# edouardoyallon/acco

Hardware: NVIDIA H100
Metric: tokens/sec (device-timed, max over ranks) Llama ACCO bf16 sharded-Adam, 8x1024 tokens per GPU per micro-batch (higher is better)
Workload: dtype bf16

## Files before the change

### acco_b200/csrc/bindings.cpp

```cpp
#include <torch/extension.h>
#include <ATen/cuda/CUDAContext.h>
#include <c10/cuda/CUDAGuard.h>
#include <cuda_runtime.h>

#include <cmath>
#include <cstdlib>
#include <vector>

extern "C" {
int acco_norm_grid(int T, int H, int sms, int backward);
int acco_norm_fwd(const void* a, const void* r, const void* w, const void* b, void* y, void* h, float* mean, float* rstd, int T, int H,
                  float eps, int grid, cudaStream_t st);
int acco_norm_bwd(const void* dy, const void* dh_extra, const void* h, const void* w, const float* mean, const float* rstd, void* dh,
                  float* partial, float* dwdb_out, void* dw_accum, void* db_accum, int T, int H, int grid, cudaStream_t st);
int acco_rope_pack_bwd(const void* dq, const void* dk, const void* dv, const long long* strides, void* dqkv, const float* cos_t,
                       const float* sin_t, int B, int S, int Hq, int Hk, int D, int sms, cudaStream_t st);
int acco_rope_qkv(void* qkv, const float* cos_t, const float* sin_t, int T, int S, int n_rot, int n_total, int D, int inverse,
                  int sms, cudaStream_t st);
int acco_swiglu_fwd(const void* gu, void* out, long long T, int I, int sms, cudaStream_t st);
int acco_swiglu_bwd(const void* dout, const void* gu, void* dgu, long long T, int I, int sms, cudaStream_t st);
int acco_ce_fwd(const void* logits, const long long* labels, float* lse, float* row_loss, float* loss, float* inv_n, long long T,
                int V, int Vp, long long ignore_index, cudaStream_t st);
int acco_ce_bwd(void* logits, const long long* labels, const float* lse, const float* scale, long long T, int V, int Vp,
                long long ignore_index, cudaStream_t st);
int acco_gelu_fwd(const void* x, void* y, long long n, int sms, cudaStream_t st);
int acco_gelu_bwd(const void* dy, const void* x, void* dx, long long n, int sms, cudaStream_t st);
int acco_debug_occupy(unsigned long long ns, int ctas, float* sink, cudaStream_t st);
int acco_round_params_size();
int acco_gemm_run(const void* a, long long lda, int a_mn, const void* b, long long ldb, int b_mn, void* d, long long ldd, const void* bias,
                  int M, int N, int K, int accumulate, int bn_req, int splits_req, int pm_req, int pn_req, int msub_req, int sms, cudaStream_t st);
int acco_gemm_tn_gather(const void* x, const void* w_local, void* y, int M, int N, int K, const void* const* peers, int n_peers,
                        const int* tile_owner, uint32_t* flags, uint32_t* epoch, uint32_t* done, int sms, cudaStream_t st);
long long acco_gemm_map_encodes();
int acco_gemm_max_clusters(int cl, int sms);
void acco_gemm_set_debug(unsigned long long* buf);
void acco_gemm_choose(int M, int N, int K, int a_mn, int b_mn, int accumulate, int sms, int* out5);
int acco_gemm_fp8_run(const void* a, long long lda, const void* b, long long ldb, void* d, long long ldd, const void* bias, int M, int N, int K,
                      int accumulate, int a_e5m2, const float* inv_a, const float* inv_b, int bn_req, int splits_req, int sms, cudaStream_t st);
int acco_fp8_amax_ctas(long long n, int sms);
int acco_fp8_quantize(const void* t, int R, int C, int e5m2, void* q, void* qT, float* scale_out, int ctas, cudaStream_t st);
int acco_gemm_tile_n();
int acco_gemm_tile_k();
int acco_attn_supported(int B, int S, int Hq, int Hk, int D, float scale);
int acco_attn_fwd(const void* q, const void* k, const void* v, long long ld, void* o, long long ld_o, float* lse, int B, int S, int Hq, int Hk,
                  int D, float scale, int window, const int* seg, cudaStream_t st);
int acco_attn_bwd(const void* q, const void* k, const void* v, long long ld, const void* o, long long ld_o, const void* d_o, long long ld_do,
                  const float* lse, float* delta, float* dq_acc, void* dk, void* dv, int B, int S, int Hq, int Hk, int D, float scale, int window,
                  const int* seg, cudaStream_t st);
}

namespace {

constexpr int kMaxWorld = 16;
struct RoundParams {
    const void* acc_peer[kMaxWorld];
    void* theta_peer[kMaxWorld];
    uint32_t* pad_peer[kMaxWorld];
    const void* acc_mc;
    void* theta_mc;
    float* master;
    float* exp_avg;
    float* exp_avg_sq;
    float* stash;
    int* stash_count;
    int* total_out;
    uint32_t* epoch;
    uint32_t* done_ctas;
    const float* inv_count_in;
    const long long* skip;
    int n_skip;
    int watchdog_s;
    int gated;
    long long slice;
    int rank, world, local_count;
    float lr, beta1, beta2, eps, weight_decay, bc1, bc2_rsqrt;
    int commit, add_stash, write_stash;
};
extern "C" int acco_rs_adam_ag(const RoundParams* P, int grad_bf16, int out_bf16, int mode, int grid, cudaStream_t st);
extern "C" int acco_round_norm(const RoundParams* P, int grad_bf16, int mode, int grid, float max_norm, float* out, cudaStream_t st);

int sm_count() {
    static int n = 0;
    if (!n) n = at::cuda::getCurrentDeviceProperties()->multiProcessorCount;
    return n;
}
cudaStream_t stream() { return at::cuda::getCurrentCUDAStream().stream(); }

void check_bf16(const torch::Tensor& t, const char* name) {
    TORCH_CHECK(t.is_cuda() && t.scalar_type() == torch::kBFloat16 && t.is_contiguous(), name, " must be a contiguous CUDA bf16 tensor");
}
void check_f32(const torch::Tensor& t, const char* name) {
    TORCH_CHECK(t.is_cuda() && t.scalar_type() == torch::kFloat32 && t.is_contiguous(), name, " must be a contiguous CUDA fp32 tensor");
}

std::vector<torch::Tensor> norm_fwd(torch::Tensor a, c10::optional<torch::Tensor> r, torch::Tensor w, c10::optional<torch::Tensor> b,
                                    double eps) {
    check_bf16(a, "a"); check_bf16(w, "weight");
    const bool has_r = r.has_value() && r->defined(), layer = b.has_value() && b->defined();
    if (has_r) check_bf16(*r, "r");
    if (layer) check_bf16(*b, "bias");
    const c10::cuda::CUDAGuard guard(a.device());
    const int T = a.size(0), H = a.size(1);
    TORCH_CHECK(w.numel() == H && (!layer || b->numel() == H), "norm: weight/bias size");
    auto y = torch::empty_like(a);
    auto f32 = a.options().dtype(torch::kFloat32);
    auto rstd = torch::empty({T}, f32);
    torch::Tensor mean = layer ? torch::empty({T}, f32) : torch::Tensor();
    torch::Tensor h = has_r ? torch::empty_like(a) : torch::Tensor();
    const int grid = acco_norm_grid(T, H, sm_count(), 0);
    TORCH_CHECK(acco_norm_fwd(a.data_ptr(), has_r ? r->data_ptr() : nullptr, w.data_ptr(), layer ? b->data_ptr() : nullptr, y.data_ptr(),
                              has_r ? h.data_ptr() : nullptr, layer ? mean.data_ptr<float>() : nullptr, rstd.data_ptr<float>(), T, H,
                              (float)eps, grid, stream()) == 0,
                "norm_fwd: unsupported hidden size ", H);
    return {y, h, mean, rstd};
}

std::vector<torch::Tensor> norm_bwd(torch::Tensor dy, c10::optional<torch::Tensor> dh_extra, torch::Tensor h, torch::Tensor w,
                                    c10::optional<torch::Tensor> mean, torch::Tensor rstd, c10::optional<torch::Tensor> wgrad,
                                    c10::optional<torch::Tensor> bgrad) {
    check_bf16(dy, "dy"); check_bf16(h, "h"); check_bf16(w, "weight"); check_f32(rstd, "rstd");
    const bool has_e = dh_extra.has_value() && dh_extra->defined(), layer = mean.has_value() && mean->defined();
    if (has_e) check_bf16(*dh_extra, "dh_extra");
    if (layer) check_f32(*mean, "mean");
    const c10::cuda::CUDAGuard guard(dy.device());
    const int T = dy.size(0), H = dy.size(1), np = layer ? 2 : 1;
    auto dh = torch::empty_like(dy);
    const int grid = acco_norm_grid(T, H, sm_count(), 1);
    auto f32 = dy.options().dtype(torch::kFloat32);
    auto partial = torch::empty({grid, np * H}, f32);
    const bool accum = wgrad.has_value() && wgrad->defined() && (!layer || (bgrad.has_value() && bgrad->defined()));
    torch::Tensor dwdb;
    if (accum) {
        check_bf16(*wgrad, "weight.grad");
        TORCH_CHECK(wgrad->numel() == H, "weight.grad has the wrong size");
        if (layer) {
            check_bf16(*bgrad, "bias.grad");
            TORCH_CHECK(bgrad->numel() == H, "bias.grad has the wrong size");
        }
        dwdb = torch::empty({0}, f32);
    } else {
        dwdb = torch::empty({np * H}, f32);
    }
    TORCH_CHECK(acco_norm_bwd(dy.data_ptr(), has_e ? dh_extra->data_ptr() : nullptr, h.data_ptr(), w.data_ptr(),
                              layer ? mean->data_ptr<float>() : nullptr, rstd.data_ptr<float>(), dh.data_ptr(), partial.data_ptr<float>(),
                              accum ? nullptr : dwdb.data_ptr<float>(), accum ? wgrad->data_ptr() : nullptr,
                              accum && layer ? bgrad->data_ptr() : nullptr, T, H, grid, stream()) == 0,
                "norm_bwd: unsupported hidden size ", H);
    return {dh, dwdb};
}

torch::Tensor gelu_fwd(torch::Tensor x) {
    check_bf16(x, "x");
    const c10::cuda::CUDAGuard guard(x.device());
    auto y = torch::empty_like(x);
    TORCH_CHECK(acco_gelu_fwd(x.data_ptr(), y.data_ptr(), x.numel(), sm_count(), stream()) == 0, "gelu: numel must be a multiple of 8");
    return y;
}
torch::Tensor gelu_bwd(torch::Tensor dy, torch::Tensor x) {
    check_bf16(x, "x"); check_bf16(dy, "dy");
    const c10::cuda::CUDAGuard guard(x.device());
    auto dx = torch::empty_like(x);
    TORCH_CHECK(acco_gelu_bwd(dy.data_ptr(), x.data_ptr(), dx.data_ptr(), x.numel(), sm_count(), stream()) == 0, "gelu: numel must be a multiple of 8");
    return dx;
}

void rope_qkv_inplace(torch::Tensor qkv, torch::Tensor cos_t, torch::Tensor sin_t, int64_t B, int64_t S, int64_t n_rot,
                      int64_t n_total, int64_t D, bool inverse) {
    check_bf16(qkv, "qkv"); check_f32(cos_t, "cos"); check_f32(sin_t, "sin");
    const c10::cuda::CUDAGuard guard(qkv.device());
    TORCH_CHECK(qkv.numel() == B * S * n_total * D, "qkv has the wrong number of elements");
    TORCH_CHECK(cos_t.size(0) >= S && cos_t.size(1) == D / 2, "cos/sin tables must be [>=S, D/2]");
    TORCH_CHECK(acco_rope_qkv(qkv.data_ptr(), cos_t.data_ptr<float>(), sin_t.data_ptr<float>(), (int)(B * S), (int)S, (int)n_rot,
                              (int)n_total, (int)D, inverse ? 1 : 0, sm_count(), stream()) == 0,
                "rope: head_dim must be a multiple of 16");
}

torch::Tensor rope_pack_bwd(torch::Tensor dq, torch::Tensor dk, torch::Tensor dv, torch::Tensor cos_t, torch::Tensor sin_t) {
    TORCH_CHECK(dq.is_cuda() && dq.scalar_type() == torch::kBFloat16 && dk.scalar_type() == torch::kBFloat16 && dv.scalar_type() == torch::kBFloat16, "bf16 CUDA grads expected");
    TORCH_CHECK(dq.stride(3) == 1 && dk.stride(3) == 1 && dv.stride(3) == 1, "head dim must be contiguous");
    check_f32(cos_t, "cos"); check_f32(sin_t, "sin");
    const c10::cuda::CUDAGuard guard(dq.device());
    const int64_t B = dq.size(0), S = dq.size(1), Hq = dq.size(2), D = dq.size(3), Hk = dk.size(2);
    for (auto* t : {&dq, &dk, &dv}) TORCH_CHECK((t->stride(0) % 8 == 0) && (t->stride(1) % 8 == 0) && (t->stride(2) % 8 == 0) && ((uintptr_t)t->data_ptr() % 16 == 0), "16-byte aligned strides required");
    auto out = torch::empty({B * S, (Hq + 2 * Hk) * D}, dq.options());
    long long st[9] = {dq.stride(0), dq.stride(1), dq.stride(2), dk.stride(0), dk.stride(1), dk.stride(2), dv.stride(0), dv.stride(1), dv.stride(2)};
    TORCH_CHECK(acco_rope_pack_bwd(dq.data_ptr(), dk.data_ptr(), dv.data_ptr(), st, out.data_ptr(), cos_t.data_ptr<float>(), sin_t.data_ptr<float>(),
                                   (int)B, (int)S, (int)Hq, (int)Hk, (int)D, sm_count(), stream()) == 0, "rope_pack_bwd: head_dim must be a multiple of 16");
    return out;
}

torch::Tensor swiglu_fwd(torch::Tensor gu) {
    check_bf16(gu, "gate_up");
    const c10::cuda::CUDAGuard guard(gu.device());
    const int64_t T = gu.size(0), I = gu.size(1) / 2;
    auto out = torch::empty({T, I}, gu.options());
    TORCH_CHECK(acco_swiglu_fwd(gu.data_ptr(), out.data_ptr(), T, (int)I, sm_count(), stream()) == 0, "swiglu: I must be a multiple of 8");
    return out;
}

torch::Tensor swiglu_bwd(torch::Tensor dout, torch::Tensor gu) {
    check_bf16(dout, "dout"); check_bf16(gu, "gate_up");
    const c10::cuda::CUDAGuard guard(gu.device());
    const int64_t T = gu.size(0), I = gu.size(1) / 2;
    auto dgu = torch::empty_like(gu);
    TORCH_CHECK(acco_swiglu_bwd(dout.data_ptr(), gu.data_ptr(), dgu.data_ptr(), T, (int)I, sm_count(), stream()) == 0, "swiglu: I must be a multiple of 8");
    return dgu;
}

std::vector<torch::Tensor> ce_fwd(torch::Tensor logits, torch::Tensor labels, int64_t V, int64_t ignore_index) {
    check_bf16(logits, "logits");
    TORCH_CHECK(labels.is_cuda() && labels.scalar_type() == torch::kInt64 && labels.is_contiguous(), "labels must be contiguous CUDA int64");
    const c10::cuda::CUDAGuard guard(logits.device());
    const int64_t T = logits.size(0), Vp = logits.size(1);
    TORCH_CHECK(labels.numel() == T, "labels/logits row mismatch");
    auto f32 = logits.options().dtype(torch::kFloat32);
    auto lse = torch::empty({T}, f32);
    auto row_loss = torch::empty({T}, f32);
    auto loss = torch::empty({}, f32);
    auto inv_n = torch::empty({1}, f32);
    TORCH_CHECK(acco_ce_fwd(logits.data_ptr(), (const long long*)labels.data_ptr<int64_t>(), lse.data_ptr<float>(), row_loss.data_ptr<float>(),
                            loss.data_ptr<float>(), inv_n.data_ptr<float>(), T, (int)V, (int)Vp, ignore_index, stream()) == 0,
                "ce_fwd: padded vocab must be a multiple of 8 and >= V");
    return {loss, inv_n, lse};
}

void ce_bwd_inplace(torch::Tensor logits, torch::Tensor labels, torch::Tensor lse, torch::Tensor scale, int64_t V, int64_t ignore_index) {
    check_bf16(logits, "logits"); check_f32(lse, "lse"); check_f32(scale, "scale");
    const c10::cuda::CUDAGuard guard(logits.device());
    const int64_t T = logits.size(0), Vp = logits.size(1);
    TORCH_CHECK(acco_ce_bwd(logits.data_ptr(), (const long long*)labels.data_ptr<int64_t>(), lse.data_ptr<float>(), scale.data_ptr<float>(), T,
                            (int)V, (int)Vp, ignore_index, stream()) == 0, "ce_bwd: bad shapes");
}

int default_grid(int mode, long long slice) {
    const long long vec = slice / 8;
    long long want = (vec + 255) / 256;
    long long cap = mode == 0 ? (long long)sm_count() * 4 : (long long)sm_count();
    if (want < 1) want = 1;
    return (int)std::min(want, cap);
}

void fill_hyper(RoundParams& P, double lr, double b1, double b2, double eps, double wd, int64_t step, int64_t commit, bool add_stash, bool write_stash) {
    P.lr = (float)lr; P.beta1 = (float)b1; P.beta2 = (float)b2; P.eps = (float)eps; P.weight_decay = (float)wd;
    P.bc1 = (float)(1.0 - std::pow(b1, (double)step));
    P.bc2_rsqrt = (float)(1.0 / std::sqrt(1.0 - std::pow(b2, (double)step)));
    P.commit = (int)commit; P.add_stash = add_stash ? 1 : 0; P.write_stash = write_stash ? 1 : 0;
}

void adamw_shard(torch::Tensor grad_sum, torch::Tensor master, torch::Tensor exp_avg, torch::Tensor exp_avg_sq, torch::Tensor stash,
                 torch::Tensor out, torch::Tensor inv_count, torch::Tensor scratch ,
                 double lr, double b1, double b2, double eps, double wd, int64_t step, int64_t commit, bool add_stash, bool write_stash) {
    check_f32(master, "master"); check_f32(exp_avg, "exp_avg"); check_f32(exp_avg_sq, "exp_avg_sq"); check_f32(stash, "stash"); check_f32(inv_count, "inv_count");
    const c10::cuda::CUDAGuard guard(master.device());
    const int64_t S = master.numel();
    TORCH_CHECK(S % 8 == 0, "shard size must be a multiple of 8 (use slice alignment >= 8)");
    TORCH_CHECK(grad_sum.numel() >= S && out.numel() >= S && grad_sum.is_contiguous() && out.is_contiguous(), "bad grad/out");
    TORCH_CHECK(scratch.scalar_type() == torch::kInt32 && scratch.numel() >= 4, "scratch must be int32[4]");
    const bool gb = grad_sum.scalar_type() == torch::kBFloat16, ob = out.scalar_type() == torch::kBFloat16;
    TORCH_CHECK(gb || grad_sum.scalar_type() == torch::kFloat32, "grad dtype");
    TORCH_CHECK(ob || out.scalar_type() == torch::kFloat32, "out dtype");
    RoundParams P{};
    P.acc_peer[0] = grad_sum.data_ptr();
    P.theta_peer[0] = out.data_ptr();
    P.master = master.data_ptr<float>(); P.exp_avg = exp_avg.data_ptr<float>(); P.exp_avg_sq = exp_avg_sq.data_ptr<float>(); P.stash = stash.data_ptr<float>();
    int* sc = scratch.data_ptr<int>();
    P.stash_count = sc; P.total_out = sc + 1; P.epoch = (uint32_t*)(sc + 2); P.done_ctas = (uint32_t*)(sc + 3);
    P.inv_count_in = inv_count.data_ptr<float>();
    P.slice = S; P.rank = 0; P.world = 1; P.local_count = 0;
    fill_hyper(P, lr, b1, b2, eps, wd, step, commit, add_stash, write_stash);
    TORCH_CHECK(acco_rs_adam_ag(&P, gb, ob, 0, default_grid(0, S), stream()) == 0, "adamw_shard launch failed");
}

RoundParams round_params(const std::vector<int64_t>& acc_ptrs, const std::vector<int64_t>& theta_ptrs, const std::vector<int64_t>& pad_ptrs,
                         int64_t acc_mc, int64_t theta_mc, const torch::Tensor& stash, const torch::Tensor& scratch, int64_t slice, int64_t rank,
                         int64_t world, int64_t local_count, int64_t mode) {
    check_f32(stash, "stash");
    TORCH_CHECK(world >= 1 && world <= kMaxWorld, "world size out of range");
    TORCH_CHECK(mode >= 0 && mode <= 2, "mode must be 0 (local), 1 (p2p) or 2 (multimem)");
    TORCH_CHECK((int64_t)acc_ptrs.size() >= (mode == 0 ? 1 : world), "peer pointer table too short");
    TORCH_CHECK(mode == 0 || (int64_t)pad_ptrs.size() >= world, "signal pad table too short");
    TORCH_CHECK(slice % 8 == 0 && stash.numel() == slice, "slice must be a multiple of 8 and match the shard state");
    TORCH_CHECK(mode != 2 || acc_mc != 0, "multicast mode needs multicast pointers");
    TORCH_CHECK(scratch.scalar_type() == torch::kInt32 && scratch.numel() >= 4, "scratch must be int32[4]");
    RoundParams P{};
    for (size_t i = 0; i < acc_ptrs.size() && i < (size_t)kMaxWorld; ++i) P.acc_peer[i] = (const void*)acc_ptrs[i];
    for (size_t i = 0; i < theta_ptrs.size() && i < (size_t)kMaxWorld; ++i) P.theta_peer[i] = (void*)theta_ptrs[i];
    for (size_t i = 0; i < pad_ptrs.size() && i < (size_t)kMaxWorld; ++i) P.pad_peer[i] = (uint32_t*)pad_ptrs[i];
    P.acc_mc = (const void*)acc_mc; P.theta_mc = (void*)theta_mc;
    P.stash = stash.data_ptr<float>();
    int* sc = scratch.data_ptr<int>();
    P.stash_count = sc; P.total_out = sc + 1; P.epoch = (uint32_t*)(sc + 2); P.done_ctas = (uint32_t*)(sc + 3);
    P.inv_count_in = nullptr;
    P.slice = slice; P.rank = (int)rank; P.world = (int)world; P.local_count = (int)local_count;
    static int watchdog = -1;
    if (watchdog < 0) { const char* e = std::getenv("ACCO_ROUND_WATCHDOG_S"); watchdog = e ? std::atoi(e) : 1800; }
    P.watchdog_s = watchdog;
    static int gated = -1;
    if (gated < 0) { const char* e = std::getenv("ACCO_ROUND_GATE"); gated = (e && e[0] == '0') ? 0 : 1; }
    P.gated = mode != 0 ? gated : 0;
    return P;
}

void rs_adam_ag(std::vector<int64_t> acc_ptrs, std::vector<int64_t> theta_ptrs, std::vector<int64_t> pad_ptrs, int64_t acc_mc, int64_t theta_mc,
                torch::Tensor master, torch::Tensor exp_avg, torch::Tensor exp_avg_sq, torch::Tensor stash,
                torch::Tensor scratch , int64_t slice, int64_t rank, int64_t world, int64_t local_count,
                double lr, double b1, double b2, double eps, double wd, int64_t step, int64_t commit, bool add_stash, bool write_stash,
                bool grad_bf16, bool out_bf16, int64_t mode, int64_t grid, c10::optional<torch::Tensor> skip_ranges,
                c10::optional<torch::Tensor> inv_count) {
    check_f32(master, "master"); check_f32(exp_avg, "exp_avg"); check_f32(exp_avg_sq, "exp_avg_sq");
    const c10::cuda::CUDAGuard guard(master.device());
    TORCH_CHECK(master.numel() == slice, "slice must match the shard state");
    TORCH_CHECK((int64_t)theta_ptrs.size() >= (mode == 0 ? 1 : world), "peer pointer tables too short");
    TORCH_CHECK(mode != 2 || theta_mc != 0, "multicast mode needs multicast pointers");
    RoundParams P = round_params(acc_ptrs, theta_ptrs, pad_ptrs, acc_mc, theta_mc, stash, scratch, slice, rank, world, local_count, mode);
    P.master = master.data_ptr<float>(); P.exp_avg = exp_avg.data_ptr<float>(); P.exp_avg_sq = exp_avg_sq.data_ptr<float>();
    if (skip_ranges.has_value() && skip_ranges->defined() && skip_ranges->numel() > 0) {
        TORCH_CHECK(skip_ranges->is_cuda() && skip_ranges->scalar_type() == torch::kInt64 && skip_ranges->is_contiguous() && skip_ranges->numel() % 2 == 0,
                    "skip_ranges must be a contiguous CUDA int64 [n, 2] tensor");
        P.skip = (const long long*)skip_ranges->data_ptr<int64_t>();
        P.n_skip = (int)(skip_ranges->numel() / 2);
    }
    if (inv_count.has_value() && inv_count->defined()) {
        check_f32(*inv_count, "inv_count");
        TORCH_CHECK(inv_count->numel() >= 2, "inv_count must be the scratch of round_norm (inv_eff at index 1)");
        P.inv_count_in = inv_count->data_ptr<float>() + 1;
        if (mode != 0) P.gated = 2;
    }
    fill_hyper(P, lr, b1, b2, eps, wd, step, commit, add_stash, write_stash);
    const int g = grid > 0 ? (int)grid : default_grid((int)mode, slice);
    TORCH_CHECK(acco_rs_adam_ag(&P, grad_bf16, out_bf16, (int)mode, g, stream()) == 0, "rs_adam_ag launch failed");
}

void round_norm(std::vector<int64_t> acc_ptrs, std::vector<int64_t> pad_ptrs, int64_t acc_mc, torch::Tensor stash, torch::Tensor scratch,
                torch::Tensor out, int64_t slice, int64_t rank, int64_t world, int64_t local_count, bool add_stash, bool grad_bf16, int64_t mode,
                int64_t grid, double max_norm) {
    check_f32(out, "out");
    const c10::cuda::CUDAGuard guard(stash.device());
    TORCH_CHECK(max_norm > 0, "max_norm must be positive");
    RoundParams P = round_params(acc_ptrs, std::vector<int64_t>(), pad_ptrs, acc_mc, 0, stash, scratch, slice, rank, world, local_count, mode);
    P.add_stash = add_stash ? 1 : 0;
    const int g = grid > 0 ? (int)grid : default_grid((int)mode, slice);
    TORCH_CHECK(out.numel() >= 3 + g, "out must hold 3 + grid floats (", 3 + g, ")");
    TORCH_CHECK(acco_round_norm(&P, grad_bf16, (int)mode, g, (float)max_norm, out.data_ptr<float>(), stream()) == 0, "round_norm launch failed");
}

torch::Tensor gemm_tn(torch::Tensor x, torch::Tensor w, std::vector<int64_t> peer_ptrs, c10::optional<torch::Tensor> tile_owner,
                      c10::optional<torch::Tensor> flags, c10::optional<torch::Tensor> state, int64_t max_ctas) {
    check_bf16(x, "x"); check_bf16(w, "w");
    TORCH_CHECK(x.dim() == 2 && w.dim() == 2 && x.size(1) == w.size(1), "gemm_tn: x [M,K], w [N,K]");
    const c10::cuda::CUDAGuard guard(x.device());
    const int64_t M = x.size(0), K = x.size(1), N = w.size(0);
    TORCH_CHECK(K % 8 == 0 && N % 8 == 0, "gemm_tn: K and N must be multiples of 8");
    TORCH_CHECK((uintptr_t)x.data_ptr() % 16 == 0 && (uintptr_t)w.data_ptr() % 16 == 0, "gemm_tn: 16-byte aligned operands required");
    auto y = torch::empty({M, N}, x.options());
    const void* peers[8] = {nullptr};
    const int n_peers = (int)peer_ptrs.size();
    TORCH_CHECK(n_peers <= 8, "gemm_tn: at most 8 peers");
    const int* owner = nullptr; uint32_t* fl = nullptr; uint32_t* ep = nullptr; uint32_t* dn = nullptr;
    if (n_peers > 0) {
        TORCH_CHECK(tile_owner.has_value() && flags.has_value() && state.has_value(), "gather mode needs tile_owner, flags and state");
        const int64_t num_n = (N + acco_gemm_tile_n() - 1) / acco_gemm_tile_n(), num_k = (K + acco_gemm_tile_k() - 1) / acco_gemm_tile_k();
        TORCH_CHECK(tile_owner->scalar_type() == torch::kInt32 && tile_owner->numel() >= num_n && tile_owner->is_cuda(), "tile_owner: int32 CUDA [num_n]");
        TORCH_CHECK(flags->scalar_type() == torch::kInt32 && flags->numel() >= num_n * num_k * 2 && flags->is_cuda(), "flags: int32 CUDA [num_n*num_k*2]");
        TORCH_CHECK(state->scalar_type() == torch::kInt32 && state->numel() >= 2 && state->is_cuda(), "state: int32 CUDA [2]");
        for (int i = 0; i < n_peers; ++i) peers[i] = (const void*)peer_ptrs[i];
        owner = tile_owner->data_ptr<int>();
        fl = (uint32_t*)flags->data_ptr<int>();
        ep = (uint32_t*)state->data_ptr<int>();
        dn = ep + 1;
    }
    int sms = sm_count();
    if (max_ctas > 0 && max_ctas < sms) sms = (int)max_ctas;
    int rc;
    if (n_peers > 0)
        rc = acco_gemm_tn_gather(x.data_ptr(), w.data_ptr(), y.data_ptr(), (int)M, (int)N, (int)K, peers, n_peers, owner, fl, ep, dn, sms, stream());
    else
        rc = acco_gemm_run(x.data_ptr(), K, 0, w.data_ptr(), K, 0, y.data_ptr(), N, nullptr, (int)M, (int)N, (int)K, 0, 0, 0, 0, 0, 0, sms, stream());
    TORCH_CHECK(rc == 0, "gemm_tn launch failed, code ", rc);
    return y;
}

torch::Tensor gemm(torch::Tensor a, torch::Tensor b, c10::optional<torch::Tensor> out, c10::optional<torch::Tensor> bias, bool a_mn, bool b_mn,
                   bool accumulate, int64_t bn, int64_t splits, int64_t pm, int64_t pn, int64_t msub, int64_t max_ctas) {
    auto ok2d = [](const torch::Tensor& t) {
        return t.is_cuda() && t.scalar_type() == torch::kBFloat16 && t.dim() == 2 && t.stride(1) == 1 && t.stride(0) % 8 == 0 && t.stride(0) >= t.size(1) &&
               (uintptr_t)t.data_ptr() % 16 == 0;
    };
    TORCH_CHECK(ok2d(a) && ok2d(b), "gemm: operands must be 2-D CUDA bf16, unit inner stride, 16-byte aligned rows");
    const c10::cuda::CUDAGuard guard(a.device());
    const int64_t M = a_mn ? a.size(1) : a.size(0), K = a_mn ? a.size(0) : a.size(1);
    const int64_t N = b_mn ? b.size(1) : b.size(0), Kb = b_mn ? b.size(0) : b.size(1);
    TORCH_CHECK(K == Kb, "gemm: contraction sizes differ (", K, " vs ", Kb, ")");
    TORCH_CHECK(N % 8 == 0, "gemm: N must be a multiple of 8");
    torch::Tensor y;
    if (out.has_value() && out->defined()) {
        y = *out;
        TORCH_CHECK(ok2d(y) && y.size(0) == M && y.size(1) == N, "gemm: out must be a [M,N] CUDA bf16 matrix");
    } else {
        TORCH_CHECK(!accumulate, "gemm: accumulate needs `out`");
        y = torch::empty({M, N}, a.options());
    }
    const void* bias_p = nullptr;
    if (bias.has_value() && bias->defined()) {
        TORCH_CHECK(bias->is_cuda() && bias->scalar_type() == torch::kBFloat16 && bias->is_contiguous() && bias->numel() == N &&
                    (uintptr_t)bias->data_ptr() % 16 == 0, "gemm: bias must be a contiguous, 16-byte aligned CUDA bf16 [N] vector");
        bias_p = bias->data_ptr();
    }
    int sms = sm_count();
    if (max_ctas > 0 && max_ctas < sms) sms = (int)max_ctas;
    const int rc = acco_gemm_run(a.data_ptr(), a.stride(0), a_mn ? 1 : 0, b.data_ptr(), b.stride(0), b_mn ? 1 : 0, y.data_ptr(), y.stride(0), bias_p,
                             (int)M, (int)N, (int)K, accumulate ? 1 : 0, (int)bn, (int)splits, (int)pm, (int)pn, (int)msub, sms, stream());
    TORCH_CHECK(rc == 0, "gemm launch failed, code ", rc, " (M=", M, " N=", N, " K=", K, ")");
    return y;
}

std::vector<torch::Tensor> fp8_quantize(torch::Tensor t, bool e5m2, bool rowmajor, bool transposed) {
    check_bf16(t, "t");
    TORCH_CHECK(t.dim() == 2 && t.size(0) % 16 == 0 && t.size(1) % 16 == 0 && t.numel() > 0, "fp8_quantize: t must be [R, C] with R, C multiples of 16");
    TORCH_CHECK((uintptr_t)t.data_ptr() % 16 == 0, "fp8_quantize: 16-byte aligned input required");
    const c10::cuda::CUDAGuard guard(t.device());
    const int64_t R = t.size(0), C = t.size(1);
    const auto f8 = t.options().dtype(e5m2 ? torch::kFloat8_e5m2 : torch::kFloat8_e4m3fn);
    torch::Tensor q = rowmajor ? torch::empty({R, C}, f8) : torch::Tensor();
    torch::Tensor qT = transposed ? torch::empty({C, R}, f8) : torch::Tensor();
    const int ctas = acco_fp8_amax_ctas(t.numel(), sm_count());
    auto scale = torch::empty({3 + ctas}, t.options().dtype(torch::kFloat32));
    TORCH_CHECK(acco_fp8_quantize(t.data_ptr(), (int)R, (int)C, e5m2 ? 1 : 0, rowmajor ? q.data_ptr() : nullptr, transposed ? qT.data_ptr() : nullptr,
                                  scale.data_ptr<float>(), ctas, stream()) == 0,
                "fp8_quantize launch failed");
    return {q, qT, scale};
}

torch::Tensor gemm_fp8(torch::Tensor a, torch::Tensor b, torch::Tensor scale_a, torch::Tensor scale_b, c10::optional<torch::Tensor> out,
                       c10::optional<torch::Tensor> bias, bool accumulate, int64_t bn, int64_t splits) {
    auto ok2d = [](const torch::Tensor& t) {
        return t.is_cuda() && t.dim() == 2 && t.stride(1) == 1 && t.stride(0) % 16 == 0 && t.stride(0) >= t.size(1) && (uintptr_t)t.data_ptr() % 16 == 0;
    };
    TORCH_CHECK(ok2d(a) && ok2d(b), "gemm_fp8: operands must be 2-D CUDA, unit inner stride, 16-byte aligned rows");
    TORCH_CHECK(a.scalar_type() == torch::kFloat8_e4m3fn || a.scalar_type() == torch::kFloat8_e5m2, "gemm_fp8: a must be e4m3 or e5m2");
    TORCH_CHECK(b.scalar_type() == torch::kFloat8_e4m3fn, "gemm_fp8: b must be e4m3");
    check_f32(scale_a, "scale_a"); check_f32(scale_b, "scale_b");
    TORCH_CHECK(scale_a.numel() >= 2 && scale_b.numel() >= 2, "gemm_fp8: scales must be {s, 1/s, ...}");
    const c10::cuda::CUDAGuard guard(a.device());
    const int64_t M = a.size(0), K = a.size(1), N = b.size(0);
    TORCH_CHECK(b.size(1) == K, "gemm_fp8: contraction sizes differ (", K, " vs ", b.size(1), ")");
    TORCH_CHECK(K % 16 == 0 && N % 8 == 0, "gemm_fp8: K must be a multiple of 16 and N of 8");
    torch::Tensor y;
    if (out.has_value() && out->defined()) {
        y = *out;
        TORCH_CHECK(y.is_cuda() && y.scalar_type() == torch::kBFloat16 && y.dim() == 2 && y.size(0) == M && y.size(1) == N && y.stride(1) == 1 &&
                    y.stride(0) % 8 == 0 && (uintptr_t)y.data_ptr() % 16 == 0, "gemm_fp8: out must be a [M,N] CUDA bf16 matrix with 16-byte aligned rows");
    } else {
        TORCH_CHECK(!accumulate, "gemm_fp8: accumulate needs `out`");
        y = torch::empty({M, N}, a.options().dtype(torch::kBFloat16));
    }
    const void* bias_p = nullptr;
    if (bias.has_value() && bias->defined()) {
        TORCH_CHECK(bias->is_cuda() && bias->scalar_type() == torch::kBFloat16 && bias->is_contiguous() && bias->numel() == N &&
                    (uintptr_t)bias->data_ptr() % 16 == 0, "gemm_fp8: bias must be a contiguous, 16-byte aligned CUDA bf16 [N] vector");
        bias_p = bias->data_ptr();
    }
    const int rc = acco_gemm_fp8_run(a.data_ptr(), a.stride(0), b.data_ptr(), b.stride(0), y.data_ptr(), y.stride(0), bias_p, (int)M, (int)N, (int)K,
                                     accumulate ? 1 : 0, a.scalar_type() == torch::kFloat8_e5m2 ? 1 : 0, scale_a.data_ptr<float>() + 1,
                                     scale_b.data_ptr<float>() + 1, (int)bn, (int)splits, sm_count(), stream());
    TORCH_CHECK(rc == 0, "gemm_fp8 launch failed, code ", rc, " (M=", M, " N=", N, " K=", K, ")");
    return y;
}

std::vector<int64_t> gemm_choose(int64_t M, int64_t N, int64_t K, bool a_mn, bool b_mn, bool accumulate) {
    int o[5] = {0, 0, 0, 0, 0};
    acco_gemm_choose((int)M, (int)N, (int)K, a_mn ? 1 : 0, b_mn ? 1 : 0, accumulate ? 1 : 0, sm_count(), o);
    return {o[0], o[1], o[2], o[3], o[4]};
}
int64_t gemm_map_encodes() { return acco_gemm_map_encodes(); }
void gemm_set_debug(c10::optional<torch::Tensor> buf) {
    if (buf.has_value() && buf->defined()) {
        TORCH_CHECK(buf->is_cuda() && buf->scalar_type() == torch::kInt64 && buf->numel() >= 16 && buf->is_contiguous(), "int64 CUDA [16] expected");
        acco_gemm_set_debug((unsigned long long*)buf->data_ptr<int64_t>());
    } else {
        acco_gemm_set_debug(nullptr);
    }
}
int64_t gemm_max_clusters(int64_t cl) { return acco_gemm_max_clusters((int)cl, sm_count()); }

int64_t num_sms() { return sm_count(); }

int64_t prefer_shared_carveout() { return (int64_t)cudaDeviceSetCacheConfig(cudaFuncCachePreferShared); }

bool attn_supported(int64_t B, int64_t S, int64_t Hq, int64_t Hk, int64_t D, double scale) {
    return acco_attn_supported((int)B, (int)S, (int)Hq, (int)Hk, (int)D, (float)scale) != 0;
}
static void check_rows(const torch::Tensor& t, int64_t rows, int64_t cols, const char* name) {
    TORCH_CHECK(t.is_cuda() && t.scalar_type() == torch::kBFloat16 && t.dim() == 2 && t.size(0) == rows && t.size(1) == cols && t.stride(1) == 1 &&
                t.stride(0) % 8 == 0 && (uintptr_t)t.data_ptr() % 16 == 0, name, " must be a [", rows, ", ", cols, "] CUDA bf16 matrix with 16-byte aligned rows");
}
static const int* seg_ptr(const c10::optional<torch::Tensor>& seg, int64_t B, int64_t S) {
    if (!seg.has_value() || !seg->defined()) return nullptr;
    TORCH_CHECK(seg->is_cuda() && seg->scalar_type() == torch::kInt32 && seg->is_contiguous() && seg->numel() == B * S,
                "seg must be a contiguous CUDA int32 tensor of B*S segment starts");
    return seg->data_ptr<int>();
}
std::vector<torch::Tensor> attn_fwd(torch::Tensor qkv, int64_t B, int64_t S, int64_t Hq, int64_t Hk, int64_t D, double scale, int64_t window,
                                    c10::optional<torch::Tensor> seg) {
    check_rows(qkv, B * S, (Hq + 2 * Hk) * D, "qkv");
    const c10::cuda::CUDAGuard guard(qkv.device());
    auto o = torch::empty({B * S, Hq * D}, qkv.options());
    auto lse = torch::empty({B, Hq, S}, qkv.options().dtype(torch::kFloat32));
    const auto* base = (const char*)qkv.data_ptr();
    const int rc = acco_attn_fwd(base, base + 2 * Hq * D, base + 2 * (Hq + Hk) * D, qkv.stride(0), o.data_ptr(), o.stride(0), lse.data_ptr<float>(), (int)B, (int)S,
                                 (int)Hq, (int)Hk, (int)D, (float)scale, (int)window, seg_ptr(seg, B, S), stream());
    TORCH_CHECK(rc == 0, "attn_fwd launch failed, code ", rc, " (B=", B, " S=", S, " Hq=", Hq, " Hk=", Hk, " D=", D, ")");
    return {o, lse};
}
std::vector<torch::Tensor> attn_bwd(torch::Tensor qkv, torch::Tensor o, torch::Tensor d_o, torch::Tensor lse, int64_t B, int64_t S, int64_t Hq, int64_t Hk,
                                    int64_t D, double scale, int64_t window, c10::optional<torch::Tensor> seg) {
    check_rows(qkv, B * S, (Hq + 2 * Hk) * D, "qkv");
    check_rows(o, B * S, Hq * D, "o");
    check_rows(d_o, B * S, Hq * D, "d_o");
    check_f32(lse, "lse");
    TORCH_CHECK(lse.numel() == B * Hq * S, "lse must be [B, Hq, S]");
    const c10::cuda::CUDAGuard guard(qkv.device());
    auto f32 = qkv.options().dtype(torch::kFloat32);
    auto delta = torch::empty({B, Hq, S}, f32);
    auto dq = torch::empty({B * S, Hq * D}, f32);
    auto dk = torch::empty({B * S, Hk * D}, qkv.options());
    auto dv = torch::empty({B * S, Hk * D}, qkv.options());
    const auto* base = (const char*)qkv.data_ptr();
    const int rc = acco_attn_bwd(base, base + 2 * Hq * D, base + 2 * (Hq + Hk) * D, qkv.stride(0), o.data_ptr(), o.stride(0), d_o.data_ptr(), d_o.stride(0),
                                 lse.data_ptr<float>(), delta.data_ptr<float>(), dq.data_ptr<float>(), dk.data_ptr(), dv.data_ptr(), (int)B, (int)S, (int)Hq,
                                 (int)Hk, (int)D, (float)scale, (int)window, seg_ptr(seg, B, S), stream());
    TORCH_CHECK(rc == 0, "attn_bwd launch failed, code ", rc);
    return {dq, dk, dv};
}

void debug_occupy(double us, int64_t ctas, torch::Tensor sink) {
    check_f32(sink, "sink");
    const c10::cuda::CUDAGuard guard(sink.device());
    TORCH_CHECK(acco_debug_occupy((unsigned long long)(us * 1e3), (int)ctas, sink.data_ptr<float>(), stream()) == 0, "occupy launch failed");
}

}

torch::Tensor pack_const_len_native(torch::Tensor flat_tokens, torch::Tensor doc_lens, int64_t max_length, int64_t eos);

PYBIND11_MODULE(TORCH_EXTENSION_NAME, m) {
    TORCH_CHECK(acco_round_params_size() == (int)sizeof(RoundParams), "RoundParams layout mismatch between bindings.cpp and rs_adam_ag.cu");
    m.def("norm_fwd", &norm_fwd);
    m.def("norm_bwd", &norm_bwd);
    m.def("gelu_fwd", &gelu_fwd);
    m.def("gelu_bwd", &gelu_bwd);
    m.def("rope_qkv_inplace", &rope_qkv_inplace);
    m.def("rope_pack_bwd", &rope_pack_bwd);
    m.def("swiglu_fwd", &swiglu_fwd);
    m.def("swiglu_bwd", &swiglu_bwd);
    m.def("ce_fwd", &ce_fwd);
    m.def("ce_bwd_inplace", &ce_bwd_inplace);
    m.def("adamw_shard", &adamw_shard);
    m.def("rs_adam_ag", &rs_adam_ag, py::arg("acc_ptrs"), py::arg("theta_ptrs"), py::arg("pad_ptrs"), py::arg("acc_mc"), py::arg("theta_mc"),
          py::arg("master"), py::arg("exp_avg"), py::arg("exp_avg_sq"), py::arg("stash"), py::arg("scratch"), py::arg("slice"), py::arg("rank"),
          py::arg("world"), py::arg("local_count"), py::arg("lr"), py::arg("b1"), py::arg("b2"), py::arg("eps"), py::arg("wd"), py::arg("step"),
          py::arg("commit"), py::arg("add_stash"), py::arg("write_stash"), py::arg("grad_bf16"), py::arg("out_bf16"), py::arg("mode"),
          py::arg("grid"), py::arg("skip_ranges"), py::arg("inv_count") = py::none());
    m.def("round_norm", &round_norm, py::arg("acc_ptrs"), py::arg("pad_ptrs"), py::arg("acc_mc"), py::arg("stash"), py::arg("scratch"),
          py::arg("out"), py::arg("slice"), py::arg("rank"), py::arg("world"), py::arg("local_count"), py::arg("add_stash"), py::arg("grad_bf16"),
          py::arg("mode"), py::arg("grid"), py::arg("max_norm"));
    m.def("gemm_tn", &gemm_tn);
    m.def("gemm", &gemm);
    m.def("gemm_choose", &gemm_choose);
    m.def("fp8_quantize", &fp8_quantize);
    m.def("gemm_fp8", &gemm_fp8);
    m.def("gemm_map_encodes", &gemm_map_encodes);
    m.def("gemm_max_clusters", &gemm_max_clusters);
    m.def("gemm_set_debug", &gemm_set_debug);
    m.def("num_sms", &num_sms);
    m.def("prefer_shared_carveout", &prefer_shared_carveout);
    m.def("attn_supported", &attn_supported);
    m.def("attn_fwd", &attn_fwd, py::arg("qkv"), py::arg("B"), py::arg("S"), py::arg("Hq"), py::arg("Hk"), py::arg("D"), py::arg("scale"),
          py::arg("window"), py::arg("seg") = py::none());
    m.def("attn_bwd", &attn_bwd, py::arg("qkv"), py::arg("o"), py::arg("d_o"), py::arg("lse"), py::arg("B"), py::arg("S"), py::arg("Hq"),
          py::arg("Hk"), py::arg("D"), py::arg("scale"), py::arg("window"), py::arg("seg") = py::none());
    m.def("debug_occupy", &debug_occupy);
    m.def("pack_const_len", &pack_const_len_native);
}
```

### acco_b200/csrc/gemm_wgmma.cu

```cuda
#include <cuda.h>
#include <cuda_bf16.h>
#include <cuda_runtime.h>
#include <stdint.h>
#include <stdlib.h>

#include <mutex>
#include <unordered_map>

#include "wgmma.cuh"

namespace acco_gemm {

using namespace acco_tc;

constexpr int BM = 128, BN_MAX = 256, BK = 64;
constexpr int A_BYTES = BM * BK * 2;
constexpr int RING_BYTES = 192 * 1024;
constexpr int MAX_STAGES = 8;
constexpr int EPI_BUF_BYTES = 64 * 64 * 2;
constexpr int EPI_BYTES = 2 * 2 * EPI_BUF_BYTES;
constexpr int SMEM_BYTES = RING_BYTES + EPI_BYTES + 1024  + 256 ;
constexpr int THREADS = 384;
constexpr int MAX_PEERS = 8;
constexpr int MN_CHUNK_BYTES = 64 * BK * 2;

struct Params {
    CUtensorMap map_a;
    CUtensorMap map_b;
    CUtensorMap map_b_peer[MAX_PEERS];
    CUtensorMap map_d;
    const __nv_bfloat16* bias;
    const int* tile_owner;
    uint32_t* flags;
    uint32_t* epoch;
    uint32_t* done_ctas;
    __nv_bfloat16* out;
    long long ldd;
    int M, N, K;
    int splits, kb_per_split;
    int reduce;
    int atomic;
    int gather;
    int stages, stage_bytes;
    int pm, pn;
    int band;
    unsigned long long* dbg;
    const float* inv_scale_a;
    const float* inv_scale_b;
};

constexpr int OP_BF16 = 0, OP_E4M3 = 1, OP_E5M2 = 2;

__device__ __forceinline__ void wait_flag_gpu(const uint32_t* f, uint32_t epoch) {
    uint32_t v;
    unsigned spins = 0;
    unsigned long long t0 = 0;
    do {
        asm volatile("ld.acquire.gpu.global.u32 %0, [%1];" : "=r"(v) : "l"(f) : "memory");
        if ((++spins & 0xFFFFF) == 0) {
            unsigned long long now;
            asm volatile("mov.u64 %0, %%globaltimer;" : "=l"(now));
            if (t0 == 0) t0 = now;
            else if (now - t0 > 60ull * 1000000000ull) __trap();
        }
    } while ((int32_t)(v - epoch) < 0);
}

__device__ __forceinline__ void stamp(const Params& P, int slot) {
    if (P.dbg != nullptr && blockIdx.x == 0) {
        unsigned long long t;
        asm volatile("mov.u64 %0, %%globaltimer;" : "=l"(t));
        P.dbg[slot] = t;
    }
}

struct Unit {
    int mb, n_blk, kb0, kb1;
};
__device__ __forceinline__ Unit decode_unit(int t, int tiles, int num_smb, int num_sn, int band, int num_k, int kb_per_split, int pm, int pn,
                                            int pi, int pj) {
    Unit u;
    const int s = t / tiles, tile = t - s * tiles;
    const int bi = tile / (band * num_smb), sn0 = bi * band;
    const int width = min(band, num_sn - sn0);
    const int r = tile - sn0 * num_smb;
    const int smb = r / width;
    u.mb = smb * pm + pi;
    u.n_blk = (sn0 + r - smb * width) * pn + pj;
    u.kb0 = s * kb_per_split;
    u.kb1 = min(num_k, u.kb0 + kb_per_split);
    return u;
}

template <int BN, int TA, int TB>
__device__ __forceinline__ void mma_k16(float (&acc)[BN / 2], uint64_t da, uint64_t db, uint32_t scale_d) {
    if constexpr (BN == 256) wgmma_m64n256k16<TA, TB>(acc, da, db, scale_d);
    else if constexpr (BN == 128) wgmma_m64n128k16<TA, TB>(acc, da, db, scale_d);
    else wgmma_m64n64k16<TA, TB>(acc, da, db, scale_d);
}

template <int BN, int OP>
__device__ __forceinline__ void mma_k32(float (&acc)[BN / 2], uint64_t da, uint64_t db, uint32_t scale_d) {
    static_assert(BN <= 128, "FP8 tiles: the promoted fragment doubles the accumulator registers");
    if constexpr (BN == 128) wgmma_m64n128k32_f8<OP == OP_E5M2>(acc, da, db, scale_d);
    else wgmma_m64n64k32_f8<OP == OP_E5M2>(acc, da, db, scale_d);
}

template <int BN, int A_MN, int B_MN, int OP>
__device__ __forceinline__ void gemm_body(const Params& P) {
    static_assert(OP == OP_BF16 || (A_MN == 0 && B_MN == 0), "FP8 wgmma has no transpose: both operands K-major");
    constexpr int BKE = OP ? 2 * BK : BK;
    extern __shared__ uint8_t smem_raw[];
    if (threadIdx.x == 0) stamp(P, 0);
    uint8_t* smem = (uint8_t*)(((uintptr_t)smem_raw + 1023) & ~(uintptr_t)1023);
    uint8_t* epi_smem = smem + RING_BYTES;
    uint64_t* full_bar = (uint64_t*)(epi_smem + EPI_BYTES);
    uint64_t* empty_bar = full_bar + MAX_STAGES;
    uint64_t* c_bar = empty_bar + MAX_STAGES;

    constexpr int B_BYTES = BN * BK * 2;
    const int wg = threadIdx.x >> 7, tid = threadIdx.x & 127;
    const int n_stages = P.stages, stage_bytes = P.stage_bytes;
    const int pm = P.pm, pn = P.pn, cl_size = pm * pn;
    const uint32_t cl_rank = cl_size > 1 ? cluster_ctarank() : 0u;
    const int pi = (int)cl_rank / pn, pj = (int)cl_rank - pi * pn;
    const int unit0 = blockIdx.x / cl_size, unit_stride = gridDim.x / cl_size;
    const int num_n = (P.N + BN - 1) / BN, num_k = (P.K + BKE - 1) / BKE, num_mb = (P.M + BM - 1) / BM;
    const int num_sn = (num_n + pn - 1) / pn, num_smb = (num_mb + pm - 1) / pm;
    const int band = P.band;
    const int tiles = num_smb * num_sn;
    const int num_units = tiles * P.splits;
    const int kbs = P.kb_per_split;
    uint16_t mask_a = 0, mask_b = 0;
    for (int j = 0; j < pn; ++j) mask_a |= (uint16_t)(1u << (pi * pn + j));
    for (int i = 0; i < pm; ++i) mask_b |= (uint16_t)(1u << (i * pn + pj));
    const uint16_t mask_rel = mask_a | mask_b;

    if (threadIdx.x == 0) {
        asm volatile("prefetch.tensormap [%0];" ::"l"(&P.map_a) : "memory");
        asm volatile("prefetch.tensormap [%0];" ::"l"(&P.map_b) : "memory");
        asm volatile("prefetch.tensormap [%0];" ::"l"(&P.map_d) : "memory");
        for (int s = 0; s < n_stages; ++s) {
            mbar_init(&full_bar[s], 1);
            mbar_init(&empty_bar[s], 2u * (uint32_t)(pm + pn - 1));
        }
        for (int b = 0; b < 4; ++b) mbar_init(&c_bar[b], 1);
        asm volatile("fence.mbarrier_init.release.cluster;" ::: "memory");
    }
    __syncthreads();
    if (cl_size > 1) cluster_sync_all();
    if (threadIdx.x == 0) stamp(P, 1);
    asm volatile("griddepcontrol.wait;" ::: "memory");
    asm volatile("griddepcontrol.launch_dependents;" ::: "memory");
    if (threadIdx.x == 0) stamp(P, 2);
    const uint32_t epoch = P.gather ? (*(volatile uint32_t*)P.epoch + 1u) : 0u;
    auto flag_ptr = [&](int n_blk, int kb, int half) { return P.flags + ((size_t)n_blk * num_k + kb) * 2 + half; };

    if (wg == 0) {
        asm volatile("setmaxnreg.dec.sync.aligned.u32 40;");
        if (tid == 0) {
            int stage = 0;
            uint32_t phase = 0;
            const int a_rows = BM / pn, a_off = pj * a_rows;
            const int nach = (BM / 64) / pn, a_ch0 = pj * nach;
            const int b_rows = BN / pm, b_off = pi * b_rows;
            const int nbch = (BN / 64) / pm, b_ch0 = pi * nbch;
            const bool mc_a = pn > 1, mc_b = pm > 1;
            for (int t = unit0; t < num_units; t += unit_stride) {
                const Unit u = decode_unit(t, tiles, num_smb, num_sn, band, num_k, kbs, pm, pn, pi, pj);
                const int n_blk = u.n_blk;
                const int m0 = u.mb * BM, n0 = n_blk * BN;
                const int owner = P.gather ? P.tile_owner[n_blk] : -1;
                const bool gatherer = owner >= 0 && u.mb == 0;
                const bool waiter = owner >= 0 && u.mb != 0;
                const CUtensorMap* bmap = gatherer ? &P.map_b_peer[owner] : &P.map_b;
                bool all_ready = !waiter;
                if (waiter) {
                    uint32_t v0, v1;
                    asm volatile("ld.acquire.gpu.global.u32 %0, [%1];" : "=r"(v0) : "l"(flag_ptr(n_blk, num_k - 1, 0)) : "memory");
                    asm volatile("ld.acquire.gpu.global.u32 %0, [%1];" : "=r"(v1) : "l"(flag_ptr(n_blk, num_k - 1, 1)) : "memory");
                    all_ready = (int32_t)(v0 - epoch) >= 0 && (int32_t)(v1 - epoch) >= 0;
                    if (all_ready) asm volatile("fence.proxy.async;" ::: "memory");
                }
                for (int kb = u.kb0; kb < u.kb1; ++kb) {
                    if (!all_ready) {
                        wait_flag_gpu(flag_ptr(n_blk, kb, 0), epoch);
                        wait_flag_gpu(flag_ptr(n_blk, kb, 1), epoch);
                        asm volatile("fence.proxy.async;" ::: "memory");
                    }
                    mbar_wait(&empty_bar[stage], phase ^ 1);
                    uint8_t* sa = smem + stage * stage_bytes;
                    uint8_t* sb = sa + A_BYTES;
                    mbar_expect_tx(&full_bar[stage], (uint32_t)(A_BYTES + B_BYTES));
                    if (A_MN) {
                        for (int c = a_ch0; c < a_ch0 + nach; ++c) {
                            if (mc_a) tma_load_2d_mc(&P.map_a, &full_bar[stage], sa + c * MN_CHUNK_BYTES, m0 + c * 64, kb * BKE, mask_a);
                            else tma_load_2d(&P.map_a, &full_bar[stage], sa + c * MN_CHUNK_BYTES, m0 + c * 64, kb * BKE);
                        }
                    } else {
                        if (mc_a) tma_load_2d_mc(&P.map_a, &full_bar[stage], sa + a_off * 128, kb * BKE, m0 + a_off, mask_a);
                        else tma_load_2d(&P.map_a, &full_bar[stage], sa, kb * BKE, m0);
                    }
                    if (B_MN) {
                        for (int c = b_ch0; c < b_ch0 + nbch; ++c) {
                            if (mc_b) tma_load_2d_mc(bmap, &full_bar[stage], sb + c * MN_CHUNK_BYTES, n0 + c * 64, kb * BKE, mask_b);
                            else tma_load_2d(bmap, &full_bar[stage], sb + c * MN_CHUNK_BYTES, n0 + c * 64, kb * BKE);
                        }
                    } else {
                        if (mc_b) tma_load_2d_mc(bmap, &full_bar[stage], sb + b_off * 128, kb * BKE, n0 + b_off, mask_b);
                        else tma_load_2d(bmap, &full_bar[stage], sb, kb * BKE, n0);
                    }
                    if (gatherer) {
                        mbar_wait(&full_bar[stage], phase);
                        fence_async_smem();
                        tma_store_2d(&P.map_b, sb, kb * BKE, n0);
                        asm volatile("cp.async.bulk.commit_group;" ::: "memory");
                        asm volatile("cp.async.bulk.wait_group 0;" ::: "memory");
                        asm volatile("fence.proxy.async;" ::: "memory");
                        asm volatile("st.release.gpu.global.u32 [%0], %1;" ::"l"(flag_ptr(n_blk, kb, 0)), "r"(epoch) : "memory");
                        asm volatile("st.release.gpu.global.u32 [%0], %1;" ::"l"(flag_ptr(n_blk, kb, 1)), "r"(epoch) : "memory");
                    }
                    if (t == unit0 && kb == u.kb0) stamp(P, 3);
                    if (++stage == n_stages) { stage = 0; phase ^= 1; }
                }
            }
            stamp(P, 9);
        }
    } else {
        asm volatile("setmaxnreg.inc.sync.aligned.u32 232;");
        const int cw = wg - 1;
        const int warp = tid >> 5, lane = tid & 31;
        const bool releaser = cl_size > 1 ? (tid < 16 && ((mask_rel >> tid) & 1)) : tid == 0;
        constexpr uint32_t a_lbo = A_MN ? (MN_CHUNK_BYTES >> 4) : 1, a_sbo = 1024 >> 4, a_kstep = A_MN ? 2048 : 32;
        constexpr uint32_t b_lbo = B_MN ? (MN_CHUNK_BYTES >> 4) : 1, b_sbo = 1024 >> 4, b_kstep = B_MN ? 2048 : 32;
        auto release = [&](int s) {
            if (!releaser) return;
            if (cl_size > 1) mbar_arrive_cluster_addr(map_to_cta(&empty_bar[s], (uint32_t)tid));
            else mbar_arrive(&empty_bar[s]);
        };
        constexpr int NSUB = BN / 64;
        constexpr int NPRE = NSUB < 2 ? NSUB : 2;
        uint8_t* epi = epi_smem + cw * 2 * EPI_BUF_BYTES;
        uint64_t* cbar = c_bar + cw * 2;
        const bool load_c = P.reduce && !P.atomic;
        const int bar_id = 1 + cw;
        uint32_t c_phase = 0;
        auto wait_buffer_free = [&]() {
            if (NSUB == 1) bulk_wait_read<0>();
            else bulk_wait_read<1>();
        };
        auto load_c_sub = [&](const Unit& u, int s) {
            mbar_expect_tx(&cbar[s & 1], (uint32_t)EPI_BUF_BYTES);
            tma_load_2d(&P.map_d, &cbar[s & 1], epi + (s & 1) * EPI_BUF_BYTES, u.n_blk * BN + s * 64, u.mb * BM + cw * 64);
        };
        float acc[BN / 2];
#pragma unroll
        for (int i = 0; i < BN / 2; ++i) acc[i] = 0.f;
        float part[OP ? BN / 2 : 1];
        float out_scale = 1.f;
        if constexpr (OP != OP_BF16) out_scale = P.inv_scale_a[0] * P.inv_scale_b[0];
        int stage = 0;
        uint32_t phase = 0;
        for (int t = unit0; t < num_units; t += unit_stride) {
            const Unit u = decode_unit(t, tiles, num_smb, num_sn, band, num_k, kbs, pm, pn, pi, pj);
            int prev = -1;
            if constexpr (OP != OP_BF16) {
#pragma unroll
                for (int i = 0; i < BN / 2; ++i) acc[i] = 0.f;
            }
            for (int kb = u.kb0; kb < u.kb1; ++kb) {
                mbar_wait(&full_bar[stage], phase);
                if (cw == 0 && tid == 0 && t == unit0 && kb == u.kb0) stamp(P, 4);
                const uint32_t a_addr = smem_u32(smem + stage * stage_bytes) + (uint32_t)(cw * 8192);
                const uint32_t b_addr = smem_u32(smem + stage * stage_bytes + A_BYTES);
                wgmma_fence();
                if constexpr (OP != OP_BF16) {
#pragma unroll
                    for (int k = 0; k < BKE / 32; ++k) {
                        const uint64_t da = make_smem_desc(a_addr + k * 32, 1, 1024 >> 4);
                        const uint64_t db = make_smem_desc(b_addr + k * 32, 1, 1024 >> 4);
                        mma_k32<BN, OP>(part, da, db, (uint32_t)(k != 0));
                    }
                } else {
#pragma unroll
                    for (int k = 0; k < BK / 16; ++k) {
                        const uint64_t da = make_smem_desc(a_addr + k * a_kstep, a_lbo, a_sbo);
                        const uint64_t db = make_smem_desc(b_addr + k * b_kstep, b_lbo, b_sbo);
                        mma_k16<BN, A_MN, B_MN>(acc, da, db, (uint32_t)((kb > u.kb0) | (k != 0)));
                    }
                }
                wgmma_commit();
                if (load_c && kb == u.kb0 && tid == 0) {
                    bulk_wait_read<0>();
                    for (int s = 0; s < NPRE; ++s) load_c_sub(u, s);
                }
                if constexpr (OP != OP_BF16) {
                    wgmma_wait<0>();
                    reg_fence(part);
                    release(stage);
#pragma unroll
                    for (int i = 0; i < BN / 2; ++i) acc[i] += part[i];
                } else {
                    if (prev >= 0) {
                        wgmma_wait<1>();
                        release(prev);
                    }
                    prev = stage;
                }
                if (++stage == n_stages) { stage = 0; phase ^= 1; }
            }
            if constexpr (OP == OP_BF16) {
                wgmma_wait<0>();
                reg_fence(acc);
                release(prev);
            }
            const int m0 = u.mb * BM + cw * 64;
            const uint32_t row_addr = smem_u32(epi) + (uint32_t)((warp * 16 + (lane >> 2)) * 128 + 4 * (lane & 3));
            const int colb = u.n_blk * BN + 2 * (lane & 3);
            const bool bias_on = P.bias != nullptr && u.kb0 == 0;
#pragma unroll
            for (int s = 0; s < NSUB; ++s) {
                uint8_t* buf = epi + (s & 1) * EPI_BUF_BYTES;
                const uint32_t buf_addr = row_addr + (uint32_t)((s & 1) * EPI_BUF_BYTES);
                if (load_c) {
                    if (s >= NPRE && tid == 0) {
                        wait_buffer_free();
                        load_c_sub(u, s);
                    }
                    mbar_wait(&cbar[s & 1], (c_phase >> (s & 1)) & 1u);
                    c_phase ^= 1u << (s & 1);
                } else {
                    if (tid == 0) wait_buffer_free();
                    named_barrier(bar_id, 128);
                }
#pragma unroll
                for (int jj = 0; jj < 8; ++jj) {
                    const int j = s * 8 + jj;
                    const int col = colb + 8 * j;
                    float b0 = 0.f, b1 = 0.f;
                    if (bias_on && col < P.N) {
                        const float2 f = __bfloat1622float2(*reinterpret_cast<const __nv_bfloat162*>(P.bias + col));
                        b0 = f.x; b1 = f.y;
                    }
                    const uint32_t chunk_addr = buf_addr + (uint32_t)((jj ^ (lane >> 2)) << 4);
#pragma unroll
                    for (int h = 0; h < 2; ++h) {
                        const uint32_t dst = chunk_addr + h * 8 * 128;
                        float v0, v1;
                        if constexpr (OP != OP_BF16) {
                            v0 = acc[4 * j + 2 * h] * out_scale + b0;
                            v1 = acc[4 * j + 2 * h + 1] * out_scale + b1;
                        } else {
                            v0 = acc[4 * j + 2 * h] + b0;
                            v1 = acc[4 * j + 2 * h + 1] + b1;
                        }
                        if (load_c) {
                            const uint32_t cv = ld_shared_u32(dst);
                            const float2 c = __bfloat1622float2(*reinterpret_cast<const __nv_bfloat162*>(&cv));
                            v0 += c.x; v1 += c.y;
                        }
                        st_shared_u32(dst, pack_bf16x2(v0, v1));
                    }
                }
                fence_async_smem();
                named_barrier(bar_id, 128);
                if (tid == 0) {
                    if (P.atomic) tma_reduce_add_2d(&P.map_d, buf, u.n_blk * BN + s * 64, m0);
                    else tma_store_2d(&P.map_d, buf, u.n_blk * BN + s * 64, m0);
                    bulk_commit();
                }
            }
        }
        if (tid == 0) bulk_wait<0>();
        if (cw == 0 && tid == 0) stamp(P, 7);
    }

    __syncthreads();
    if (threadIdx.x == 0) stamp(P, 10);
    if (cl_size > 1) cluster_sync_all();
    if (P.gather && threadIdx.x == 0) {
        __threadfence();
        const uint32_t prev = atomicAdd(P.done_ctas, 1u);
        if (prev == gridDim.x - 1) {
            *P.done_ctas = 0;
            __threadfence();
            *P.epoch = epoch;
        }
    }
}

template <int BN, int A_MN, int B_MN>
__global__ void __launch_bounds__(THREADS, 1) gemm_kernel(const __grid_constant__ Params P) {
    gemm_body<BN, A_MN, B_MN, OP_BF16>(P);
}

template <int BN, int OP>
__global__ void __launch_bounds__(THREADS, 1) gemm_fp8_kernel(const __grid_constant__ Params P) {
    gemm_body<BN, 0, 0, OP>(P);
}

typedef CUresult (*EncodeFn)(CUtensorMap*, CUtensorMapDataType, cuuint32_t, void*, const cuuint64_t*, const cuuint64_t*, const cuuint32_t*,
                             const cuuint32_t*, CUtensorMapInterleave, CUtensorMapSwizzle, CUtensorMapL2promotion, CUtensorMapFloatOOBfill);

static EncodeFn get_encode() {
    static EncodeFn fn = nullptr;
    static std::once_flag once;
    std::call_once(once, [] {
        void* p = nullptr;
        cudaDriverEntryPointQueryResult q;
        if (cudaGetDriverEntryPoint("cuTensorMapEncodeTiled", &p, cudaEnableDefault, &q) == cudaSuccess) fn = (EncodeFn)p;
    });
    return fn;
}

static bool bind_primary_context() {
    typedef CUresult (*DeviceGetFn)(CUdevice*, int);
    typedef CUresult (*RetainFn)(CUcontext*, CUdevice);
    typedef CUresult (*SetCurrentFn)(CUcontext);
    void *p_get = nullptr, *p_retain = nullptr, *p_set = nullptr;
    cudaDriverEntryPointQueryResult q;
    if (cudaGetDriverEntryPoint("cuDeviceGet", &p_get, cudaEnableDefault, &q) != cudaSuccess ||
        cudaGetDriverEntryPoint("cuDevicePrimaryCtxRetain", &p_retain, cudaEnableDefault, &q) != cudaSuccess ||
        cudaGetDriverEntryPoint("cuCtxSetCurrent", &p_set, cudaEnableDefault, &q) != cudaSuccess)
        return false;
    int dev = 0;
    CUdevice d;
    CUcontext c = nullptr;
    if (cudaGetDevice(&dev) != cudaSuccess || ((DeviceGetFn)p_get)(&d, dev) != CUDA_SUCCESS) return false;
    return ((RetainFn)p_retain)(&c, d) == CUDA_SUCCESS && ((SetCurrentFn)p_set)(c) == CUDA_SUCCESS;
}

struct MapKey {
    const void* base;
    uint64_t inner, outer, ld;
    uint32_t box_inner, box_outer;
    int elem_bytes;
    bool operator==(const MapKey& o) const {
        return base == o.base && inner == o.inner && outer == o.outer && ld == o.ld && box_inner == o.box_inner && box_outer == o.box_outer &&
               elem_bytes == o.elem_bytes;
    }
};
struct MapKeyHash {
    size_t operator()(const MapKey& k) const {
        size_t h = (size_t)k.base;
        auto mix = [&h](uint64_t v) { h ^= v + 0x9e3779b97f4a7c15ull + (h << 6) + (h >> 2); };
        mix(k.inner); mix(k.outer); mix(k.ld); mix(((uint64_t)k.box_inner << 32) | k.box_outer); mix((uint64_t)k.elem_bytes);
        return h;
    }
};
static std::mutex g_map_mu;
static std::unordered_map<MapKey, CUtensorMap, MapKeyHash> g_maps;
static long long g_map_encodes = 0;

int make_map_typed(CUtensorMap* m, const void* base, uint64_t inner, uint64_t outer, uint64_t ld, uint32_t box_inner, uint32_t box_outer,
                   int elem_bytes) {
    const MapKey key{base, inner, outer, ld, box_inner, box_outer, elem_bytes};
    {
        std::lock_guard<std::mutex> g(g_map_mu);
        auto it = g_maps.find(key);
        if (it != g_maps.end()) { *m = it->second; return 0; }
    }
    EncodeFn enc = get_encode();
    if (!enc) return -2;
    cuuint64_t dims[2] = {inner, outer};
    cuuint64_t strides[1] = {ld * (uint64_t)elem_bytes};
    cuuint32_t box[2] = {box_inner, box_outer};
    cuuint32_t estr[2] = {1, 1};
    const CUtensorMapDataType dt = elem_bytes == 4 ? CU_TENSOR_MAP_DATA_TYPE_FLOAT32
                                   : elem_bytes == 1 ? CU_TENSOR_MAP_DATA_TYPE_UINT8 : CU_TENSOR_MAP_DATA_TYPE_BFLOAT16;
    CUresult r = enc(m, dt, 2, const_cast<void*>(base), dims, strides, box, estr, CU_TENSOR_MAP_INTERLEAVE_NONE,
                     CU_TENSOR_MAP_SWIZZLE_128B, CU_TENSOR_MAP_L2_PROMOTION_L2_256B, CU_TENSOR_MAP_FLOAT_OOB_FILL_NONE);
    if (r == CUDA_ERROR_INVALID_CONTEXT && bind_primary_context()) {
        r = enc(m, dt, 2, const_cast<void*>(base), dims, strides, box, estr,
                CU_TENSOR_MAP_INTERLEAVE_NONE, CU_TENSOR_MAP_SWIZZLE_128B, CU_TENSOR_MAP_L2_PROMOTION_L2_256B, CU_TENSOR_MAP_FLOAT_OOB_FILL_NONE);
    }
    if (r != CUDA_SUCCESS) return -3;
    std::lock_guard<std::mutex> g(g_map_mu);
    if (g_maps.size() > 8192) g_maps.clear();
    g_maps.emplace(key, *m);
    ++g_map_encodes;
    return 0;
}
static int make_map(CUtensorMap* m, const void* base, uint64_t inner, uint64_t outer, uint64_t ld, uint32_t box_inner, uint32_t box_outer) {
    return make_map_typed(m, base, inner, outer, ld, box_inner, box_outer, 2);
}

typedef void (*KernelFn)(const Params);
template <int BN>
static KernelFn kernel_for(int a_mn, int b_mn) {
    if (a_mn) return b_mn ? gemm_kernel<BN, 1, 1> : gemm_kernel<BN, 1, 0>;
    return b_mn ? gemm_kernel<BN, 0, 1> : gemm_kernel<BN, 0, 0>;
}
static KernelFn kernel_for(int bn, int a_mn, int b_mn) {
    if (bn == 256) return kernel_for<256>(a_mn, b_mn);
    if (bn == 128) return kernel_for<128>(a_mn, b_mn);
    return kernel_for<64>(a_mn, b_mn);
}
static KernelFn fp8_kernel_for(int bn, int op) {
    if (bn == 128) return op == OP_E5M2 ? gemm_fp8_kernel<128, OP_E5M2> : gemm_fp8_kernel<128, OP_E4M3>;
    return op == OP_E5M2 ? gemm_fp8_kernel<64, OP_E5M2> : gemm_fp8_kernel<64, OP_E4M3>;
}

static int g_pm = 0, g_pn = 0;
static unsigned long long* g_dbg = nullptr;
static int g_pdl = 1;
static int init_once() {
    static int rc = 0;
    static std::once_flag once;
    std::call_once(once, [] {
        for (int bn : {64, 128, 256})
            for (int a = 0; a < 2; ++a)
                for (int b = 0; b < 2; ++b)
                    if (cudaFuncSetAttribute(kernel_for(bn, a, b), cudaFuncAttributeMaxDynamicSharedMemorySize, SMEM_BYTES) != cudaSuccess) rc = -4;
        for (int bn : {64, 128})
            for (int op : {OP_E4M3, OP_E5M2})
                if (cudaFuncSetAttribute(fp8_kernel_for(bn, op), cudaFuncAttributeMaxDynamicSharedMemorySize, SMEM_BYTES) != cudaSuccess) rc = -4;
        const char* e;
        if ((e = getenv("ACCO_GEMM_CLUSTER")) && e[0] && e[1] == ',') { g_pm = e[0] - '0'; g_pn = e[2] - '0'; }
        if ((e = getenv("ACCO_GEMM_PDL")) && e[0] == '0') g_pdl = 0;
    });
    return rc;
}

static int max_clusters(int cl, int sms) {
    static int cache[17] = {0};
    static std::mutex mu;
    std::lock_guard<std::mutex> g(mu);
    if (cl < 2 || cl > 16) return sms;
    if (!cache[cl]) {
        cudaLaunchConfig_t cfg = {};
        cfg.gridDim = dim3(cl * 64);
        cfg.blockDim = dim3(THREADS);
        cfg.dynamicSmemBytes = SMEM_BYTES;
        cudaLaunchAttribute attr[1];
        attr[0].id = cudaLaunchAttributeClusterDimension;
        attr[0].val.clusterDim.x = cl;
        attr[0].val.clusterDim.y = 1;
        attr[0].val.clusterDim.z = 1;
        cfg.attrs = attr;
        cfg.numAttrs = 1;
        int n = 0;
        if (cudaOccupancyMaxActiveClusters(&n, gemm_kernel<256, 0, 0>, &cfg) != cudaSuccess || n <= 0) { cudaGetLastError(); n = -1; }
        cache[cl] = n;
    }
    const int n = cache[cl];
    if (n <= 0) return 0;
    return n < sms / cl ? n : sms / cl;
}

struct Config {
    int bn, splits, pm, pn;
};

static Config choose_config(int M, int N, int K, int a_mn, int b_mn, int reduce, int sms, int bn_req, int splits_req, int pm_req, int pn_req,
                            int bn_max = BN_MAX) {
    (void)a_mn; (void)b_mn;
    const int num_k = (K + BK - 1) / BK;
    double best = 1e30;
    Config bc{bn_max, 1, 1, 1};
    const int cands[3] = {256, 128, 64};
    const int num_mb = (M + BM - 1) / BM;
    for (int ci = 0; ci < 3; ++ci) {
        const int bn = cands[ci];
        if (bn_req > 0 && bn != bn_req) continue;
        if (bn > bn_max) continue;
        if (bn_req <= 0 && bn > 64 && bn / 2 >= N) continue;
        const int num_n = (N + bn - 1) / bn;
        for (int pm = 1; pm <= 2; ++pm) {
            for (int pn = 1; pn <= 2; ++pn) {
                if ((pm_req > 0 && pm != pm_req) || (pm_req <= 0 && pm != 1)) continue;
                if ((pn_req > 0 && pn != pn_req) || (pn_req <= 0 && pn != 1)) continue;
                if (b_mn ? ((bn / 64) % pm != 0) : ((bn / pm) % 8 != 0)) continue;
                if (a_mn && (BM / 64) % pn != 0) continue;
                const int cl = pm * pn;
                const int slots = cl > 1 ? max_clusters(cl, sms) * cl : sms;
                if (slots <= 0) continue;
                const long long tiles = (long long)((num_mb + pm - 1) / pm) * ((num_n + pn - 1) / pn) * cl;
                const int max_s = reduce ? 16 : (num_k >= 128 ? 4 : 1);
                for (int s = 1; s <= max_s; ++s) {
                    if (splits_req > 0 && s != 1) break;
                    int sp = splits_req > 0 ? splits_req : s;
                    if (sp > num_k) sp = num_k;
                    const int kbs = (num_k + sp - 1) / sp;
                    if (splits_req <= 0 && s > 1 && kbs < 8) break;
                    const int s_eff = (num_k + kbs - 1) / kbs;
                    if (splits_req <= 0 && s_eff != s) continue;
                    const long long units = tiles * s_eff;
                    const long long waves = (units + slots - 1) / slots;
                    const double feed = (A_BYTES / (double)pn + bn * BK * 2 / (double)pm) / 64.0;
                    const double mma = 4.0 * bn;
                    const double per_kb = feed > mma ? feed : mma;
                    const double epi = 128.0 * bn * 2.0 / 16.0 + 800.0;
                    const double unit = kbs * per_kb + 600.0 + epi;
                    double cost = waves * unit + 1000.0 * (cl > 1);
                    if (reduce && s_eff > 1) cost += 0.05 * unit * s_eff + (double)M * N * s_eff * 4.0 / 3000.0;
                    if (!reduce && s_eff > 1) cost += 3000.0 + (double)M * N * 2.0 / 2000.0 + (double)M * N * s_eff * 4.0 / 3000.0;
                    if (cost < best) { best = cost; bc = Config{bn, s_eff, pm, pn}; }
                }
            }
        }
    }
    return bc;
}

static int tile_band(int M, int K, int bn_cols, int num_sn) {
    static int l2_cache[64] = {0};
    int dev = 0;
    if (cudaGetDevice(&dev) != cudaSuccess || dev < 0 || dev >= 64) { cudaGetLastError(); return num_sn; }
    if (l2_cache[dev] == 0) {
        int l2 = 0;
        if (cudaDeviceGetAttribute(&l2, cudaDevAttrL2CacheSize, dev) != cudaSuccess || l2 <= 0) { cudaGetLastError(); l2 = -1; }
        l2_cache[dev] = l2;
    }
    const double l2 = (double)l2_cache[dev];
    if (l2 <= 0 || (double)M * K * 2.0 > l2 / 3.0) return num_sn;
    const long long g = (long long)(l2 / 8.0 / ((double)bn_cols * K * 2.0));
    return (int)(g < 1 ? 1 : (g > num_sn ? num_sn : g));
}

struct GatherArgs {
    const void* const* peers;
    int n_peers;
    const int* tile_owner;
    uint32_t* flags;
    uint32_t* epoch;
    uint32_t* done;
};

static int launch(const void* a, long long lda, int a_mn, const void* b, long long ldb, int b_mn, void* d, long long ldd, const void* bias, int M,
                  int N, int K, int accumulate, int bn_req, int splits_req, int pm_req, int pn_req, int msub_req, const GatherArgs* ga, int sms,
                  cudaStream_t st, int op = OP_BF16, const float* inv_a = nullptr, const float* inv_b = nullptr) {
    if (M <= 0 || N <= 0 || K <= 0) return -1;
    if ((lda % 8) || (ldb % 8) || (ldd % 8) || (N % 8)) return -1;
    const int eb = op ? 1 : 2, bke = op ? 2 * BK : BK;
    if (op && (a_mn || b_mn || (lda % 16) || (ldb % 16) || (K % 16) || bn_req > 128 || !inv_a || !inv_b || (ga && ga->n_peers > 0))) return -1;
    if (((uintptr_t)a % 16) || ((uintptr_t)b % 16) || ((uintptr_t)d % 16) || (bias && ((uintptr_t)bias % 16))) return -1;
    if (msub_req > 1) return -1;
    int rc = init_once();
    if (rc) return rc;
    const int gather = (ga && ga->n_peers > 0) ? 1 : 0;
    if (gather && (ga->n_peers > MAX_PEERS || a_mn || b_mn || accumulate)) return -1;
    if (bn_req > 0 && bn_req != 64 && bn_req != 128 && bn_req != 256) return -1;
    if ((pm_req > 2) || (pn_req > 2)) return -1;
    Config cfgc{BN_MAX, 1, 1, 1};
    if (!gather) {
        if (g_pm > 0 && pm_req <= 0) pm_req = g_pm;
        if (g_pn > 0 && pn_req <= 0) pn_req = g_pn;
        cfgc = choose_config(M, N, op ? (K + 1) / 2 : K, a_mn, b_mn, accumulate, sms, bn_req, splits_req, pm_req, pn_req, op ? 128 : BN_MAX);
    }
    const int bn = cfgc.bn, pm = cfgc.pm, pn = cfgc.pn;
    int splits = cfgc.splits;
    if ((bn_req > 0 && bn != bn_req) || (pm_req > 0 && pm != pm_req) || (pn_req > 0 && pn != pn_req)) return -1;
    if (b_mn ? ((bn / 64) % pm != 0) : ((bn / pm) % 8 != 0)) return -1;
    if (a_mn && (BM / 64) % pn != 0) return -1;
    Params P;
    if (a_mn) rc = make_map(&P.map_a, a, (uint64_t)M, (uint64_t)K, (uint64_t)lda, 64, BK);
    else rc = make_map_typed(&P.map_a, a, (uint64_t)K, (uint64_t)M, (uint64_t)lda, bke, (uint32_t)(BM / pn), eb);
    if (rc) return rc;
    if (b_mn) rc = make_map(&P.map_b, b, (uint64_t)N, (uint64_t)K, (uint64_t)ldb, 64, BK);
    else rc = make_map_typed(&P.map_b, b, (uint64_t)K, (uint64_t)N, (uint64_t)ldb, bke, (uint32_t)(bn / pm), eb);
    if (rc) return rc;
    for (int i = 0; i < MAX_PEERS; ++i) {
        if (gather && i < ga->n_peers) {
            rc = make_map(&P.map_b_peer[i], ga->peers[i], (uint64_t)K, (uint64_t)N, (uint64_t)ldb, BK, (uint32_t)bn);
            if (rc) return rc;
        } else {
            P.map_b_peer[i] = P.map_b;
        }
    }
    rc = make_map(&P.map_d, d, (uint64_t)N, (uint64_t)M, (uint64_t)ldd, 64, 64);
    if (rc) return rc;
    P.bias = (const __nv_bfloat16*)bias;
    P.out = (__nv_bfloat16*)d;
    P.ldd = ldd;
    P.dbg = g_dbg;
    P.inv_scale_a = inv_a;
    P.inv_scale_b = inv_b;
    P.tile_owner = gather ? ga->tile_owner : nullptr;
    P.flags = gather ? ga->flags : nullptr;
    P.epoch = gather ? ga->epoch : nullptr;
    P.done_ctas = gather ? ga->done : nullptr;
    P.M = M; P.N = N; P.K = K;
    const int num_k = (K + bke - 1) / bke;
    if (splits < 1) splits = 1;
    if (splits > num_k) splits = num_k;
    P.kb_per_split = (num_k + splits - 1) / splits;
    P.splits = (num_k + P.kb_per_split - 1) / P.kb_per_split;
    P.reduce = accumulate ? 1 : 0;
    bool pdl = g_pdl != 0;
    if (P.splits > 1 && !P.reduce) {
        if (cudaMemset2DAsync(d, (size_t)ldd * 2, 0, (size_t)N * 2, (size_t)M, st) != cudaSuccess) return -6;
        P.reduce = 1;
        pdl = false;
    }
    P.atomic = P.splits > 1 ? 1 : 0;
    P.gather = gather;
    P.pm = pm; P.pn = pn;
    P.stage_bytes = A_BYTES + bn * BK * 2;
    P.stages = RING_BYTES / P.stage_bytes;
    if (P.stages > MAX_STAGES) P.stages = MAX_STAGES;
    const int num_n = (N + bn - 1) / bn;
    const int num_mb = (M + BM - 1) / BM;
    const int cl = pm * pn;
    const int num_sn = (num_n + pn - 1) / pn;
    const long long units = (long long)((num_mb + pm - 1) / pm) * num_sn * P.splits;
    const int slots = cl > 1 ? max_clusters(cl, sms) : sms;
    if (slots <= 0) return -5;
    P.band = gather ? num_sn : tile_band(M, op ? (K + 1) / 2 : K, bn * pn, num_sn);
    const int grid = (int)(units < (long long)slots ? units : (long long)slots) * cl;
    cudaLaunchConfig_t cfg = {};
    cfg.gridDim = dim3(grid);
    cfg.blockDim = dim3(THREADS);
    cfg.dynamicSmemBytes = SMEM_BYTES;
    cfg.stream = st;
    cudaLaunchAttribute attr[2];
    int na = 0;
    if (cl > 1) {
        attr[na].id = cudaLaunchAttributeClusterDimension;
        attr[na].val.clusterDim.x = cl;
        attr[na].val.clusterDim.y = 1;
        attr[na].val.clusterDim.z = 1;
        ++na;
    }
    if (pdl) {
        attr[na].id = cudaLaunchAttributeProgrammaticStreamSerialization;
        attr[na].val.programmaticStreamSerializationAllowed = 1;
        ++na;
    }
    cfg.attrs = attr;
    cfg.numAttrs = na;
    return (int)cudaLaunchKernelEx(&cfg, op ? fp8_kernel_for(bn, op) : kernel_for(bn, a_mn, b_mn), P);
}

}

extern "C" int acco_gemm_run(const void* a, long long lda, int a_mn, const void* b, long long ldb, int b_mn, void* d, long long ldd, const void* bias,
                             int M, int N, int K, int accumulate, int bn_req, int splits_req, int pm_req, int pn_req, int msub_req, int sms,
                             cudaStream_t st) {
    return acco_gemm::launch(a, lda, a_mn, b, ldb, b_mn, d, ldd, bias, M, N, K, accumulate, bn_req, splits_req, pm_req, pn_req, msub_req, nullptr, sms,
                             st);
}

extern "C" int acco_gemm_tn_gather(const void* x, const void* w_local, void* y, int M, int N, int K, const void* const* peers, int n_peers,
                                   const int* tile_owner, uint32_t* flags, uint32_t* epoch, uint32_t* done, int sms, cudaStream_t st) {
    acco_gemm::GatherArgs ga{peers, n_peers, tile_owner, flags, epoch, done};
    return acco_gemm::launch(x, K, 0, w_local, K, 0, y, N, nullptr, M, N, K, 0, 0, 0, 0, 0, 0, n_peers > 0 ? &ga : nullptr, sms, st);
}

extern "C" int acco_gemm_fp8_run(const void* a, long long lda, const void* b, long long ldb, void* d, long long ldd, const void* bias, int M, int N,
                                 int K, int accumulate, int a_e5m2, const float* inv_a, const float* inv_b, int bn_req, int splits_req, int sms,
                                 cudaStream_t st) {
    return acco_gemm::launch(a, lda, 0, b, ldb, 0, d, ldd, bias, M, N, K, accumulate, bn_req, splits_req, 0, 0, 0, nullptr, sms, st,
                             a_e5m2 ? acco_gemm::OP_E5M2 : acco_gemm::OP_E4M3, inv_a, inv_b);
}

extern "C" int acco_gemm_tile_n() { return acco_gemm::BN_MAX; }
extern "C" int acco_gemm_tile_k() { return acco_gemm::BK; }
extern "C" long long acco_gemm_map_encodes() { return acco_gemm::g_map_encodes; }
extern "C" void acco_gemm_set_debug(unsigned long long* buf) { acco_gemm::g_dbg = buf; }
extern "C" int acco_gemm_max_clusters(int cl, int sms) {
    acco_gemm::init_once();
    return acco_gemm::max_clusters(cl, sms);
}
extern "C" void acco_gemm_choose(int M, int N, int K, int a_mn, int b_mn, int accumulate, int sms, int* out5) {
    const acco_gemm::Config c = acco_gemm::choose_config(M, N, K, a_mn, b_mn, accumulate, sms, 0, 0, acco_gemm::g_pm, acco_gemm::g_pn);
    out5[0] = c.bn; out5[1] = c.splits; out5[2] = c.pm; out5[3] = c.pn; out5[4] = 1;
}
```

### acco_b200/models/llama.py

```python
from __future__ import annotations

from collections import OrderedDict
from dataclasses import dataclass, asdict
from typing import Any, Dict, Optional

import torch
import torch.nn as nn

from .. import ops
from .output import CausalLMOutput

__all__ = ["LlamaConfig", "LlamaForCausalLM"]


@dataclass
class LlamaConfig:
    vocab_size: int = 50257
    hidden_size: int = 768
    intermediate_size: int = 2048
    num_hidden_layers: int = 12
    num_attention_heads: int = 12
    num_key_value_heads: Optional[int] = None
    max_position_embeddings: int = 1024
    rms_norm_eps: float = 1e-5
    rope_theta: float = 10000.0
    rope_scaling: Optional[Dict[str, Any]] = None
    tie_word_embeddings: bool = True
    initializer_range: float = 0.02
    pad_vocab_multiple: int = 128
    model_type: str = "llama"

    def __post_init__(self):
        if self.num_key_value_heads is None:
            self.num_key_value_heads = self.num_attention_heads
        assert self.hidden_size % self.num_attention_heads == 0
        assert self.num_attention_heads % self.num_key_value_heads == 0

    @property
    def head_dim(self) -> int:
        return self.hidden_size // self.num_attention_heads

    @property
    def padded_vocab(self) -> int:
        m = max(int(self.pad_vocab_multiple), 1)
        return ((self.vocab_size + m - 1) // m) * m

    def to_dict(self) -> Dict[str, Any]:
        return asdict(self)

    @classmethod
    def from_dict(cls, d: Dict[str, Any]) -> "LlamaConfig":
        keys = cls.__dataclass_fields__.keys()
        return cls(**{k: v for k, v in dict(d).items() if k in keys})

    def num_parameters(self, padded: bool = False) -> int:
        H, I, L = self.hidden_size, self.intermediate_size, self.num_hidden_layers
        D, Hq, Hk = self.head_dim, self.num_attention_heads, self.num_key_value_heads
        V = self.padded_vocab if padded else self.vocab_size
        per_layer = (Hq + 2 * Hk) * D * H + H * Hq * D + 3 * H * I + 2 * H
        n = V * H + L * per_layer + H
        if not self.tie_word_embeddings:
            n += V * H
        return n

    def flops_per_token(self, seq_len: int) -> float:
        H, I, L = self.hidden_size, self.intermediate_size, self.num_hidden_layers
        D, Hq, Hk = self.head_dim, self.num_attention_heads, self.num_key_value_heads
        mm = L * ((Hq + 2 * Hk) * D * H + Hq * D * H + 3 * H * I) + self.vocab_size * H
        attn = L * 2 * Hq * D * seq_len / 2
        return 3.0 * 2.0 * (mm + attn)


class _Norm(nn.Module):
    def __init__(self, dim: int):
        super().__init__()
        self.weight = nn.Parameter(torch.ones(dim))


class _Attn(nn.Module):
    def __init__(self, cfg: LlamaConfig):
        super().__init__()
        D, Hq, Hk, H = cfg.head_dim, cfg.num_attention_heads, cfg.num_key_value_heads, cfg.hidden_size
        self.qkv_proj = nn.Parameter(torch.empty((Hq + 2 * Hk) * D, H))
        self.o_proj = nn.Parameter(torch.empty(H, Hq * D))


class _MLP(nn.Module):
    def __init__(self, cfg: LlamaConfig):
        super().__init__()
        self.gate_up_proj = nn.Parameter(torch.empty(2 * cfg.intermediate_size, cfg.hidden_size))
        self.down_proj = nn.Parameter(torch.empty(cfg.hidden_size, cfg.intermediate_size))


class _Layer(nn.Module):
    def __init__(self, cfg: LlamaConfig):
        super().__init__()
        self.input_layernorm = _Norm(cfg.hidden_size)
        self.self_attn = _Attn(cfg)
        self.post_attention_layernorm = _Norm(cfg.hidden_size)
        self.mlp = _MLP(cfg)


class _Body(nn.Module):
    def __init__(self, cfg: LlamaConfig):
        super().__init__()
        self.embed_tokens = nn.Parameter(torch.empty(cfg.padded_vocab, cfg.hidden_size))
        self.layers = nn.ModuleList([_Layer(cfg) for _ in range(cfg.num_hidden_layers)])
        self.norm = _Norm(cfg.hidden_size)


class LlamaForCausalLM(nn.Module):
    def __init__(self, config: LlamaConfig):
        super().__init__()
        self.config = config
        self.model = _Body(config)
        if config.tie_word_embeddings:
            self.lm_head = None
        else:
            self.lm_head = nn.Parameter(torch.empty(config.padded_vocab, config.hidden_size))
        self._rope_cache: Dict[Any, Any] = {}
        self._ag_table: Dict[int, Any] = {}
        self._ag_idx = 0
        self._ag_pending = False
        self.fp8 = False
        self.reset_parameters()

    @torch.no_grad()
    def reset_parameters(self) -> None:
        std = self.config.initializer_range
        V = self.config.vocab_size
        for name, p in self.named_parameters():
            if name.endswith("layernorm.weight") or name.endswith("norm.weight"):
                p.fill_(1.0)
            else:
                p.normal_(0.0, std)
        self.model.embed_tokens[V:].zero_()
        if self.lm_head is not None:
            self.lm_head[V:].zero_()

    @property
    def head_weight(self) -> torch.Tensor:
        return self.model.embed_tokens if self.lm_head is None else self.lm_head

    def num_parameters(self) -> int:
        return sum(p.numel() for p in self.parameters())

    def _rope(self, S: int, device) -> Any:
        key = (S, str(device))
        if key not in self._rope_cache:
            self._rope_cache[key] = ops.rope_tables(S, self.config.head_dim, self.config.rope_theta, device, scaling=self.config.rope_scaling)
        return self._rope_cache[key]

    def fused_ag_candidates(self):
        out = []
        for layer in self.model.layers:
            out += [layer.self_attn.qkv_proj, layer.self_attn.o_proj, layer.mlp.gate_up_proj, layer.mlp.down_proj]
        if self.lm_head is not None:
            out.append(self.lm_head)
        return out

    def _gw(self, p):
        if not self._ag_pending:
            return None
        e = self._ag_table.get(id(p))
        return None if e is None else e[self._ag_idx]

    def forward(self, input_ids: torch.Tensor, attention_mask: Optional[torch.Tensor] = None,
                labels: Optional[torch.Tensor] = None, position_ids: Optional[torch.Tensor] = None, **unused) -> CausalLMOutput:
        cfg = self.config
        B, S = input_ids.shape
        T = B * S
        D, Hq, Hk = cfg.head_dim, cfg.num_attention_heads, cfg.num_key_value_heads
        cos, sin = self._rope(S, input_ids.device)
        seg = None
        if position_ids is not None:
            pos = position_ids.reshape(T)
            cos, sin = cos[pos], sin[pos]
            seg = ops.segment_starts(position_ids)
        eps = cfg.rms_norm_eps
        fp8 = self.fp8

        h = ops.embedding(input_ids.reshape(T), self.model.embed_tokens)
        branch = None
        for layer in self.model.layers:
            if branch is None:
                n = ops.rmsnorm(h, layer.input_layernorm.weight, eps)
            else:
                n, h = ops.add_rmsnorm(branch, h, layer.input_layernorm.weight, eps)
            qkv = ops.linear(n, layer.self_attn.qkv_proj, gathered=self._gw(layer.self_attn.qkv_proj), fp8=fp8)
            att = ops.rope_causal_attention(qkv, cos, sin, B, S, Hq, Hk, D, seg=seg)
            o = ops.linear(att, layer.self_attn.o_proj, gathered=self._gw(layer.self_attn.o_proj), fp8=fp8)
            n, h = ops.add_rmsnorm(o, h, layer.post_attention_layernorm.weight, eps)
            gu = ops.linear(n, layer.mlp.gate_up_proj, gathered=self._gw(layer.mlp.gate_up_proj), fp8=fp8)
            branch = ops.linear(ops.swiglu(gu), layer.mlp.down_proj, gathered=self._gw(layer.mlp.down_proj), fp8=fp8)
        if branch is None:
            n = ops.rmsnorm(h, self.model.norm.weight, eps)
        else:
            n, h = ops.add_rmsnorm(branch, h, self.model.norm.weight, eps)
        logits = ops.linear(n, self.head_weight, gathered=self._gw(self.head_weight) if self.lm_head is not None else None)
        if labels is None:
            return CausalLMOutput(loss=None, logits=logits.view(B, S, -1)[..., : cfg.vocab_size])
        shifted = torch.full_like(labels, -100)
        shifted[:, :-1] = labels[:, 1:]
        loss = ops.softmax_cross_entropy(logits, shifted.reshape(T), cfg.vocab_size, -100)
        return CausalLMOutput(loss=loss, logits=None)

    def state_dict(self, *args, destination=None, prefix: str = "", keep_vars: bool = False, **kw):
        cfg = self.config
        D, Hq, Hk, V, I = cfg.head_dim, cfg.num_attention_heads, cfg.num_key_value_heads, cfg.vocab_size, cfg.intermediate_size
        get = (lambda p: p) if keep_vars else (lambda p: p.detach())
        sd = destination if destination is not None else OrderedDict()
        sd[prefix + "model.embed_tokens.weight"] = get(self.model.embed_tokens)[:V]
        for i, layer in enumerate(self.model.layers):
            base = f"{prefix}model.layers.{i}."
            qkv = get(layer.self_attn.qkv_proj)
            sd[base + "self_attn.q_proj.weight"] = qkv[: Hq * D]
            sd[base + "self_attn.k_proj.weight"] = qkv[Hq * D: (Hq + Hk) * D]
            sd[base + "self_attn.v_proj.weight"] = qkv[(Hq + Hk) * D:]
            sd[base + "self_attn.o_proj.weight"] = get(layer.self_attn.o_proj)
            gu = get(layer.mlp.gate_up_proj)
            sd[base + "mlp.gate_proj.weight"] = gu[:I]
            sd[base + "mlp.up_proj.weight"] = gu[I:]
            sd[base + "mlp.down_proj.weight"] = get(layer.mlp.down_proj)
            sd[base + "input_layernorm.weight"] = get(layer.input_layernorm.weight)
            sd[base + "post_attention_layernorm.weight"] = get(layer.post_attention_layernorm.weight)
        sd[prefix + "model.norm.weight"] = get(self.model.norm.weight)
        sd[prefix + "lm_head.weight"] = get(self.head_weight)[:V]
        return sd

    @torch.no_grad()
    def load_state_dict(self, state_dict, strict: bool = True, assign: bool = False):
        cfg = self.config
        D, Hq, Hk, V, I = cfg.head_dim, cfg.num_attention_heads, cfg.num_key_value_heads, cfg.vocab_size, cfg.intermediate_size
        sd = dict(state_dict)
        used = set()

        def take(name):
            used.add(name)
            return sd[name]

        missing = []

        def put(dst: torch.Tensor, name: str):
            if name in sd:
                dst.copy_(take(name).to(dst.dtype))
            else:
                missing.append(name)

        put(self.model.embed_tokens[:V], "model.embed_tokens.weight")
        for i, layer in enumerate(self.model.layers):
            b = f"model.layers.{i}."
            qkv, gu = layer.self_attn.qkv_proj, layer.mlp.gate_up_proj
            put(qkv[: Hq * D], b + "self_attn.q_proj.weight")
            put(qkv[Hq * D: (Hq + Hk) * D], b + "self_attn.k_proj.weight")
            put(qkv[(Hq + Hk) * D:], b + "self_attn.v_proj.weight")
            put(layer.self_attn.o_proj, b + "self_attn.o_proj.weight")
            put(gu[:I], b + "mlp.gate_proj.weight")
            put(gu[I:], b + "mlp.up_proj.weight")
            put(layer.mlp.down_proj, b + "mlp.down_proj.weight")
            put(layer.input_layernorm.weight, b + "input_layernorm.weight")
            put(layer.post_attention_layernorm.weight, b + "post_attention_layernorm.weight")
        put(self.model.norm.weight, "model.norm.weight")
        if self.lm_head is not None:
            put(self.lm_head[:V], "lm_head.weight")
        elif "lm_head.weight" in sd:
            used.add("lm_head.weight")
        unexpected = [k for k in sd if k not in used and not k.endswith("rotary_emb.inv_freq")]
        if strict and (missing or unexpected):
            raise RuntimeError(f"load_state_dict: missing={missing[:5]} unexpected={unexpected[:5]}")
        return torch.nn.modules.module._IncompatibleKeys(missing, unexpected)
```

### acco_b200/ops/__init__.py

```python
from __future__ import annotations

import glob
import importlib.util
import os
import threading
from typing import Dict, Optional

import torch

_EXT = None
_EXT_ERR: Optional[BaseException] = None
_LOCK = threading.Lock()
_PKG_DIR = os.path.dirname(os.path.dirname(os.path.abspath(__file__)))

_launch_counts: Dict[str, int] = {}
_counting = True


def count_launch(name: str, n: int = 1) -> None:
    if _counting:
        _launch_counts[name] = _launch_counts.get(name, 0) + n


def launch_counts() -> Dict[str, int]:
    return dict(_launch_counts)


def reset_launch_counts() -> None:
    _launch_counts.clear()


def total_launches() -> int:
    return sum(_launch_counts.values())


def ext_path() -> Optional[str]:
    cands = sorted(glob.glob(os.path.join(_PKG_DIR, "_C*.so")))
    return cands[-1] if cands else None


def load_ext(required: bool = False):
    global _EXT, _EXT_ERR
    if _EXT is not None:
        return _EXT
    with _LOCK:
        if _EXT is not None:
            return _EXT
        path = ext_path()
        if path is None:
            _EXT_ERR = FileNotFoundError(
                f"acco_b200/_C*.so not found under {_PKG_DIR}; run `python -c 'import __graft_entry__ as g; g.build()'`")
        else:
            try:
                spec = importlib.util.spec_from_file_location("acco_b200._C", path)
                mod = importlib.util.module_from_spec(spec)
                spec.loader.exec_module(mod)
                _EXT = mod
                _EXT_ERR = None
            except BaseException as e:
                _EXT_ERR = e
        if _EXT is None and required:
            raise RuntimeError(f"acco_b200 CUDA extension unavailable: {_EXT_ERR}")
        return _EXT


def have_ext() -> bool:
    return load_ext() is not None


def use_kernels(*tensors: torch.Tensor, bf16_only: bool = True) -> bool:
    if not tensors or not all(t.is_cuda for t in tensors if t is not None):
        return False
    if bf16_only and any(t.is_floating_point() and t.dtype != torch.bfloat16 for t in tensors if t is not None):
        return False
    if os.environ.get("ACCO_FORCE_EAGER") == "1":
        return False
    if load_ext() is not None:
        return True
    if os.environ.get("ACCO_ALLOW_FALLBACK") == "1":
        return False
    raise RuntimeError(
        "acco_b200: CUDA tensors given but the sm_90a extension is not built/loaded "
        f"({_EXT_ERR}). Build it with __graft_entry__.build() or set ACCO_ALLOW_FALLBACK=1.")


from .norm import rmsnorm, add_rmsnorm, rmsnorm_ref, add_rmsnorm_ref, layernorm, add_layernorm, layernorm_ref, add_layernorm_ref
from .rope import rope_qkv, rope_qkv_ref, apply_rope_ref, rope_tables
from .embedding import embedding
from .activation import swiglu, swiglu_ref, gelu_new, gelu_new_ref
from .cross_entropy import softmax_cross_entropy, softmax_cross_entropy_ref
from .linear import linear, LinearFn
from .attention import causal_attention, causal_attention_ref, rope_causal_attention, packed_causal_attention, segment_starts
from .adam import fused_adamw_shard, grad_sumsq

__all__ = [
    "load_ext", "have_ext", "use_kernels", "ext_path",
    "count_launch", "launch_counts", "reset_launch_counts", "total_launches",
    "rmsnorm", "add_rmsnorm", "rmsnorm_ref", "add_rmsnorm_ref",
    "layernorm", "add_layernorm", "gelu_new", "layernorm_ref", "add_layernorm_ref", "gelu_new_ref",
    "rope_qkv", "rope_qkv_ref", "apply_rope_ref", "rope_tables", "embedding",
    "swiglu", "swiglu_ref",
    "softmax_cross_entropy", "softmax_cross_entropy_ref",
    "linear", "LinearFn",
    "causal_attention", "causal_attention_ref", "rope_causal_attention", "packed_causal_attention", "segment_starts",
    "fused_adamw_shard", "grad_sumsq",
]
```

### acco_b200/ops/attention.py

```python
from __future__ import annotations

import logging
import math
import os
from typing import Optional, Tuple

import torch
import torch.nn.functional as F

_SDPA_BACKENDS = None


def _sdpa_ctx():
    global _SDPA_BACKENDS
    from torch.nn.attention import SDPBackend, sdpa_kernel
    if _SDPA_BACKENDS is None:
        _SDPA_BACKENDS = [SDPBackend.CUDNN_ATTENTION, SDPBackend.FLASH_ATTENTION, SDPBackend.EFFICIENT_ATTENTION, SDPBackend.MATH]
    try:
        return sdpa_kernel(_SDPA_BACKENDS, set_priority=True)
    except TypeError:
        return sdpa_kernel(_SDPA_BACKENDS)


def _window_mask(S: int, window: int, device) -> torch.Tensor:
    i = torch.arange(S, device=device)[:, None]
    j = torch.arange(S, device=device)[None, :]
    return (j <= i) & (j > i - window)


def segment_starts(position_ids: torch.Tensor) -> torch.Tensor:
    S = position_ids.shape[1]
    s = torch.arange(S, device=position_ids.device, dtype=position_ids.dtype)
    return (s[None, :] - position_ids).to(torch.int32).reshape(-1)


def _seg_mask(seg: torch.Tensor, B: int, S: int, window: Optional[int]) -> torch.Tensor:
    seg = seg.view(B, S).long()
    kv = torch.arange(S, device=seg.device)[None, None, :]
    vis = _window_mask(S, window if window else S, seg.device)[None] & (kv >= seg[:, :, None])
    return vis[:, None]


def causal_attention_ref(q, k, v, scale: Optional[float] = None, window: Optional[int] = None, seg: Optional[torch.Tensor] = None):
    B, S, Hq, D = q.shape
    Hk = k.shape[2]
    qf, kf, vf = (t.float().transpose(1, 2) for t in (q, k, v))
    if Hk != Hq:
        kf = kf.repeat_interleave(Hq // Hk, dim=1)
        vf = vf.repeat_interleave(Hq // Hk, dim=1)
    sc = (1.0 / math.sqrt(D)) if scale is None else scale
    att = qf @ kf.transpose(-1, -2) * sc
    mask = _window_mask(S, window if window else S, q.device) if seg is None else _seg_mask(seg, B, S, window)
    att = att.masked_fill(~mask, float("-inf")).softmax(-1)
    return (att @ vf).transpose(1, 2).to(q.dtype)


def causal_attention(q, k, v, scale: Optional[float] = None, window: Optional[int] = None, seg: Optional[torch.Tensor] = None):
    B, S, Hq, D = q.shape
    Hk = k.shape[2]
    if window is not None and window >= S:
        window = None
    if seg is not None:
        o = _attend(q.transpose(1, 2), k.transpose(1, 2), v.transpose(1, 2), scale, window, Hk != Hq, seg)
        return o.transpose(1, 2).contiguous()
    if q.is_cuda and window is not None:
        try:
            from flash_attn import flash_attn_func
            return flash_attn_func(q, k, v, softmax_scale=scale, causal=True, window_size=(window - 1, 0))
        except Exception:
            pass
    qt, kt, vt = q.transpose(1, 2), k.transpose(1, 2), v.transpose(1, 2)
    kw = {}
    if Hk != Hq:
        kw["enable_gqa"] = True
    if window is None:
        if q.is_cuda:
            with _sdpa_ctx():
                o = F.scaled_dot_product_attention(qt, kt, vt, is_causal=True, scale=scale, **kw)
        else:
            o = F.scaled_dot_product_attention(qt, kt, vt, is_causal=True, scale=scale, **kw)
    else:
        mask = _window_mask(S, window, q.device)
        o = F.scaled_dot_product_attention(qt, kt, vt, attn_mask=mask, scale=scale, **kw)
    return o.transpose(1, 2).contiguous()


def own_attention_enabled() -> bool:
    return os.environ.get("ACCO_ATTN", "").lower() == "own"


_BLK = 128
_LOG2E = 1.4426950408889634
_LN2 = 0.6931471805599453


def _bf16_round(t: torch.Tensor) -> torch.Tensor:
    return t.to(torch.bfloat16).float()


def _block_mask(q0: int, kv0: int, window: int, device, seg_row: Optional[torch.Tensor] = None) -> torch.Tensor:
    q = torch.arange(q0, q0 + _BLK, device=device)[:, None]
    kv = torch.arange(kv0, kv0 + _BLK, device=device)[None, :]
    vis = (kv <= q) & (kv + window > q)
    if seg_row is not None:
        vis = vis & (kv >= seg_row[q0:q0 + _BLK, None].long())
    return vis


def fwd_key_blocks(qb: int, S: int, window: int) -> range:
    lo = qb * _BLK - window + 1
    return range(lo // _BLK if lo > 0 else 0, qb + 1)


def bwd_query_blocks(n: int, S: int, window: int) -> range:
    return range(n, min(S // _BLK - 1, (n * _BLK + _BLK - 2 + window) // _BLK) + 1)


def fwd_key_blocks_seg(qb: int, window: int, seg_row, bq: int = _BLK, bk: int = _BLK) -> range:
    q0 = qb * bq
    lo = max(0, q0 - window + 1, int(seg_row[q0]))
    return range(lo // bk, (q0 + bq - 1) // bk + 1)


def bwd_query_blocks_seg(n: int, S: int, window: int, seg_row, bq: int = _BLK, bk: int = _BLK) -> range:
    kv0 = n * bk
    m_hi = min(S // bq - 1, (kv0 + bk - 1 + window - 1) // bq)
    m = kv0 // bq
    while m <= m_hi and int(seg_row[max(m * bq, kv0)]) <= kv0 + bk - 1:
        m += 1
    return range(kv0 // bq, m)


def attention_blockwise_ref(q, k, v, scale: Optional[float] = None, window: Optional[int] = None,
                            seg: Optional[torch.Tensor] = None) -> Tuple[torch.Tensor, torch.Tensor]:
    B, S, Hq, D = q.shape
    Hk = k.shape[2]
    assert S % _BLK == 0 and Hq % Hk == 0
    sc = (1.0 / math.sqrt(D)) if scale is None else float(scale)
    c = sc * _LOG2E
    win = S if (window is None or window <= 0 or window > S) else int(window)
    o = torch.empty(B, S, Hq, D, dtype=torch.float32, device=q.device)
    lse = torch.empty(B, Hq, S, dtype=torch.float32, device=q.device)
    for b in range(B):
        seg_row = None if seg is None else seg.view(B, S)[b]
        for h in range(Hq):
            g = h // (Hq // Hk)
            for qb in range(S // _BLK):
                q0 = qb * _BLK
                Q = q[b, q0:q0 + _BLK, h].float()
                m_run = torch.full((_BLK,), -1e30)
                l_run = torch.zeros(_BLK)
                O = torch.zeros(_BLK, D)
                pending = None
                for j in (fwd_key_blocks(qb, S, win) if seg_row is None else fwd_key_blocks_seg(qb, win, seg_row)):
                    kv0 = j * _BLK
                    Sraw = Q @ k[b, kv0:kv0 + _BLK, g].float().T
                    vis = _block_mask(q0, kv0, win, q.device, seg_row)
                    mx = Sraw.masked_fill(~vis, float("-inf")).max(dim=1).values
                    m_new = torch.maximum(m_run, mx * c)
                    alpha = torch.exp2(m_run - m_new)
                    if pending is not None:
                        O = (O + pending) * alpha[:, None]
                    l_run = l_run * alpha
                    m_run = m_new
                    Pm = torch.exp2(Sraw * c - m_new[:, None]).masked_fill(~vis, 0.0)
                    l_run = l_run + Pm.sum(dim=1)
                    pending = _bf16_round(Pm) @ v[b, kv0:kv0 + _BLK, g].float()
                O = (O + pending) / l_run[:, None]
                o[b, q0:q0 + _BLK, h] = O
                lse[b, h, q0:q0 + _BLK] = (m_run + torch.log2(l_run)) * _LN2
    return o.to(q.dtype), lse


def attention_blockwise_bwd_ref(q, k, v, o, d_o, lse, scale: Optional[float] = None, window: Optional[int] = None,
                                seg: Optional[torch.Tensor] = None):
    B, S, Hq, D = q.shape
    Hk = k.shape[2]
    G = Hq // Hk
    sc = (1.0 / math.sqrt(D)) if scale is None else float(scale)
    c = sc * _LOG2E
    win = S if (window is None or window <= 0 or window > S) else int(window)
    nqb = S // _BLK
    delta = (d_o.float() * o.float()).sum(-1).permute(0, 2, 1)
    dq = torch.zeros(B, S, Hq, D, dtype=torch.float32, device=q.device)
    dk = torch.empty(B, S, Hk, D, dtype=torch.float32, device=q.device)
    dv = torch.empty(B, S, Hk, D, dtype=torch.float32, device=q.device)
    for b in range(B):
        seg_row = None if seg is None else seg.view(B, S)[b]
        for g in range(Hk):
            for n in range(nqb):
                kv0 = n * _BLK
                K = k[b, kv0:kv0 + _BLK, g].float()
                V = v[b, kv0:kv0 + _BLK, g].float()
                dK = torch.zeros(_BLK, D)
                dV = torch.zeros(_BLK, D)
                for gi in range(G):
                    hq = g * G + gi
                    for m in (bwd_query_blocks(n, S, win) if seg_row is None else bwd_query_blocks_seg(n, S, win, seg_row)):
                        q0 = m * _BLK
                        Q = q[b, q0:q0 + _BLK, hq].float()
                        dO = d_o[b, q0:q0 + _BLK, hq].float()
                        L2 = lse[b, hq, q0:q0 + _BLK] * _LOG2E
                        dl = delta[b, hq, q0:q0 + _BLK]
                        vis = _block_mask(q0, kv0, win, q.device, seg_row)
                        Pm = torch.exp2((Q @ K.T) * c - L2[:, None]).masked_fill(~vis, 0.0)
                        dS = Pm * ((dO @ V.T) - dl[:, None]) * sc
                        Pb, dSb = _bf16_round(Pm), _bf16_round(dS)
                        dV += Pb.T @ dO
                        dK += dSb.T @ Q
                        dq[b, q0:q0 + _BLK, hq] += dSb @ K
                dk[b, kv0:kv0 + _BLK, g] = dK
                dv[b, kv0:kv0 + _BLK, g] = dV
    return dq, dk.to(q.dtype), dv.to(q.dtype)



def _sdpa(qt, kt, vt, scale, gqa: bool):
    kw = {"enable_gqa": True} if gqa else {}
    if qt.is_cuda:
        with _sdpa_ctx():
            return F.scaled_dot_product_attention(qt, kt, vt, is_causal=True, scale=scale, **kw)
    return F.scaled_dot_product_attention(qt, kt, vt, is_causal=True, scale=scale, **kw)


def _attend(q, k, v, scale, window, gqa: bool, seg: Optional[torch.Tensor] = None):
    B, S = q.shape[0], q.shape[2]
    if seg is not None:
        kw = {"enable_gqa": True} if gqa else {}
        return F.scaled_dot_product_attention(q, k, v, attn_mask=_seg_mask(seg, B, S, window), scale=scale, **kw)
    if window is not None and window < S:
        if q.is_cuda:
            try:
                from flash_attn import flash_attn_func
                o = flash_attn_func(q.transpose(1, 2), k.transpose(1, 2), v.transpose(1, 2), softmax_scale=scale, causal=True,
                                    window_size=(window - 1, 0))
                return o.transpose(1, 2)
            except ImportError:
                pass
        kw = {"enable_gqa": True} if gqa else {}
        return F.scaled_dot_product_attention(q, k, v, attn_mask=_window_mask(S, window, q.device), scale=scale, **kw)
    kw = {"enable_gqa": True} if gqa else {}
    if q.is_cuda:
        with _sdpa_ctx():
            return F.scaled_dot_product_attention(q, k, v, is_causal=True, scale=scale, **kw)
    return F.scaled_dot_product_attention(q, k, v, is_causal=True, scale=scale, **kw)


_IDENT_TABLES = {}


def _identity_tables(S: int, D: int, device):
    key = (S, D, str(device))
    if key not in _IDENT_TABLES:
        _IDENT_TABLES[key] = (torch.ones(S, D // 2, device=device, dtype=torch.float32), torch.zeros(S, D // 2, device=device, dtype=torch.float32))
    return _IDENT_TABLES[key]


_SEG_FALLBACK_LOGGED = False


def _log_seg_fallback(B, S, Hq, Hk, D) -> None:
    global _SEG_FALLBACK_LOGGED
    if not _SEG_FALLBACK_LOGGED:
        _SEG_FALLBACK_LOGGED = True
        logging.getLogger("acco_b200").warning(
            f"packed rows: the own attention kernels do not cover B={B} S={S} Hq={Hq} Hk={Hk} head_dim={D} "
            "(head_dim 64 and S % 128 == 0 needed); document masking runs on SDPA with a dense [B, 1, S, S] mask")


class _RopeAttentionFn(torch.autograd.Function):

    @staticmethod
    def forward(ctx, qkv, cos, sin, B, S, Hq, Hk, D, rope=True, scale=None, window=None, seg=None):
        from . import count_launch, load_ext
        C = load_ext(required=True)
        rb, rs = (1, B * S) if (rope and seg is not None) else (B, S)
        if rope:
            C.rope_qkv_inplace(qkv, cos, sin, rb, rs, Hq + Hk, Hq + 2 * Hk, D, False)
            count_launch("rope_qkv")
        sc = (1.0 / math.sqrt(D)) if scale is None else float(scale)
        ctx.dims = (B, S, Hq, Hk, D, rb, rs)
        ctx.save_for_backward(cos, sin)
        if (seg is not None or own_attention_enabled()) and C.attn_supported(B, S, Hq, Hk, D, sc):
            extra = () if seg is None else (seg,)
            o, lse = C.attn_fwd(qkv.detach(), B, S, Hq, Hk, D, sc, int(window or 0), *extra)
            count_launch("attn_fwd" if seg is None else "attn_fwd_seg")
            ctx.inner = None
            ctx.own = (qkv.detach(), o, lse, sc, int(window or 0), seg)
            return o
        if seg is not None:
            _log_seg_fallback(B, S, Hq, Hk, D)
        ctx.own = None
        x = qkv.detach().view(B, S, Hq + 2 * Hk, D)
        with torch.enable_grad():
            q = x[:, :, :Hq].transpose(1, 2).requires_grad_()
            k = x[:, :, Hq:Hq + Hk].transpose(1, 2).requires_grad_()
            v = x[:, :, Hq + Hk:].transpose(1, 2).requires_grad_()
            out = _attend(q, k, v, scale, window, Hk != Hq, seg)
        ctx.inner = (out, q, k, v)
        return out.detach().transpose(1, 2).reshape(B * S, Hq * D)

    @staticmethod
    def backward(ctx, dout):
        from . import count_launch, load_ext
        C = load_ext(required=True)
        cos, sin = ctx.saved_tensors
        B, S, Hq, Hk, D, rb, rs = ctx.dims
        if ctx.own is not None:
            qkv, o, lse, sc, window, seg = ctx.own
            ctx.own = None
            extra = () if seg is None else (seg,)
            dq, dk, dv = C.attn_bwd(qkv, o, dout.contiguous(), lse, B, S, Hq, Hk, D, sc, window, *extra)
            count_launch("attn_bwd" if seg is None else "attn_bwd_seg", 2)
            dqkv = C.rope_pack_bwd(dq.to(torch.bfloat16).view(rb, rs, Hq, D), dk.view(rb, rs, Hk, D), dv.view(rb, rs, Hk, D), cos, sin)
            count_launch("rope_pack_bwd")
            return (dqkv,) + (None,) * 11
        out, q, k, v = ctx.inner
        ctx.inner = None
        do = dout.reshape(B, S, Hq, D).transpose(1, 2)
        dq, dk, dv = torch.autograd.grad(out, (q, k, v), do)
        dq, dk, dv = (t if t.stride(-1) == 1 else t.contiguous() for t in (dq, dk, dv))
        dq, dk, dv = (t.transpose(1, 2) for t in (dq, dk, dv))
        if rb != B:
            dq, dk, dv = (t.reshape(rb, rs, t.shape[2], D) for t in (dq, dk, dv))
        dqkv = C.rope_pack_bwd(dq, dk, dv, cos, sin)
        count_launch("rope_pack_bwd")
        return (dqkv,) + (None,) * 11


def rope_causal_attention(qkv: torch.Tensor, cos: torch.Tensor, sin: torch.Tensor, B: int, S: int, Hq: int, Hk: int, D: int,
                          seg: Optional[torch.Tensor] = None) -> torch.Tensor:
    from . import use_kernels
    from .rope import rope_qkv_ref
    if use_kernels(qkv):
        if seg is not None or (torch.is_grad_enabled() and qkv.requires_grad):
            return _RopeAttentionFn.apply(qkv, cos, sin, B, S, Hq, Hk, D, True, None, None, seg)
        from . import count_launch, load_ext
        load_ext(required=True).rope_qkv_inplace(qkv, cos, sin, B, S, Hq + Hk, Hq + 2 * Hk, D, False)
        count_launch("rope_qkv")
        x = qkv.view(B, S, Hq + 2 * Hk, D)
        out = _sdpa(x[:, :, :Hq].transpose(1, 2), x[:, :, Hq:Hq + Hk].transpose(1, 2), x[:, :, Hq + Hk:].transpose(1, 2), None, Hk != Hq)
        return out.transpose(1, 2).reshape(B * S, Hq * D)
    if seg is None:
        x = rope_qkv_ref(qkv, cos, sin, B, S, Hq, Hk, D)
    else:
        x = rope_qkv_ref(qkv, cos, sin, 1, B * S, Hq, Hk, D)
    x = x.view(B, S, Hq + 2 * Hk, D)
    return causal_attention(x[:, :, :Hq], x[:, :, Hq:Hq + Hk], x[:, :, Hq + Hk:], seg=seg).reshape(B * S, Hq * D)


def packed_causal_attention(qkv: torch.Tensor, B: int, S: int, Hq: int, Hk: int, D: int, scale=None, window=None,
                            seg: Optional[torch.Tensor] = None) -> torch.Tensor:
    from . import use_kernels
    if use_kernels(qkv) and D % 16 == 0 and (seg is not None or (torch.is_grad_enabled() and qkv.requires_grad)):
        cos, sin = _identity_tables(S, D, qkv.device)
        return _RopeAttentionFn.apply(qkv, cos, sin, B, S, Hq, Hk, D, False, scale, window, seg)
    x = qkv.view(B, S, Hq + 2 * Hk, D)
    return causal_attention(x[:, :, :Hq], x[:, :, Hq:Hq + Hk], x[:, :, Hq + Hk:], scale=scale, window=window,
                            seg=seg).reshape(B * S, Hq * D)
```

### acco_b200/ops/linear.py

```python
from __future__ import annotations

from typing import Optional

import os

import torch
import torch.nn.functional as F


def _tc(*mats) -> bool:
    from . import use_kernels
    from .gemm import gemm_supported
    if os.environ.get("ACCO_GEMM", "") == "cublas":
        return False
    return use_kernels(*mats) and gemm_supported(*mats)


class LinearFn(torch.autograd.Function):
    @staticmethod
    @torch.amp.custom_fwd(device_type="cuda")
    def forward(ctx, x, weight, bias, accumulate_into_grad):
        ctx.save_for_backward(x, weight)
        ctx.has_bias = bias is not None
        ctx.accumulate = bool(accumulate_into_grad)
        ctx.weight_ref = weight
        ctx.bias_ref = bias
        x2 = x.reshape(-1, x.shape[-1])
        if _tc(x2, weight) and (bias is None or (bias.dtype == torch.bfloat16 and bias.data_ptr() % 16 == 0)):
            from .gemm import gemm_tn
            return gemm_tn(x2, weight.detach(), bias=None if bias is None else bias.detach()).view(*x.shape[:-1], weight.shape[0])
        return F.linear(x, weight, bias)

    @staticmethod
    @torch.amp.custom_bwd(device_type="cuda")
    def backward(ctx, dy):
        return _linear_backward(ctx, dy)


_SIDE_STREAMS = {}


def _wgrad_stream(device):
    if os.environ.get("ACCO_WGRAD_STREAM", "0") != "1" or device.type != "cuda":
        return None
    key = (device.index, torch.cuda.current_stream(device).cuda_stream)
    st = _SIDE_STREAMS.get(key)
    if st is None:
        st = _SIDE_STREAMS[key] = torch.cuda.Stream(device=device)
    return st


def _linear_backward(ctx, dy):
    x, weight = ctx.saved_tensors
    dy2 = dy.reshape(-1, dy.shape[-1])
    x2 = x.reshape(-1, x.shape[-1])
    if dy2.dtype != weight.dtype or x2.dtype != dy2.dtype:
        weight_c, x2 = weight.to(dy2.dtype), x2.to(dy2.dtype)
    else:
        weight_c = weight
    tc = _tc(dy2, weight_c, x2)
    w = ctx.weight_ref
    acc_tc = (ctx.needs_input_grad[1] and ctx.accumulate and w.grad is not None and tc and w.grad.dtype == torch.bfloat16
              and w.grad.dim() == 2 and w.grad.stride(1) == 1 and w.grad.data_ptr() % 16 == 0)
    dx = dw = None
    side = _wgrad_stream(dy2.device) if (acc_tc and ctx.needs_input_grad[0]) else None
    if side is not None:
        from .gemm import gemm_tt_acc
        cur = torch.cuda.current_stream(dy2.device)
        side.wait_stream(cur)
        with torch.cuda.stream(side):
            gemm_tt_acc(dy2, x2, w.grad)
        dy2.record_stream(side)
        x2.record_stream(side)
    if ctx.needs_input_grad[0]:
        if tc:
            from .gemm import gemm_nn
            dx = gemm_nn(dy2, weight_c.detach()).view(x.shape)
        else:
            dx = dy2.matmul(weight_c).view(x.shape).to(x.dtype)
    if side is not None:
        torch.cuda.current_stream(dy2.device).wait_stream(side)
    elif ctx.needs_input_grad[1]:
        if ctx.accumulate and w.grad is not None:
            if acc_tc:
                from .gemm import gemm_tt_acc
                gemm_tt_acc(dy2, x2, w.grad)
            elif w.grad.dtype == dy2.dtype:
                w.grad.addmm_(dy2.t(), x2)
            else:
                w.grad.add_(dy2.t().matmul(x2))
        elif tc:
            from .gemm import gemm
            dw = gemm(dy2, x2, a_mn=True, b_mn=True)
        else:
            dw = dy2.t().matmul(x2).to(weight.dtype)
    return dx, dw, _bias_grad(ctx, dy2), None


def _bias_grad(ctx, dy2):
    if not (ctx.has_bias and ctx.needs_input_grad[2]):
        return None
    b = ctx.bias_ref
    if ctx.accumulate and b.grad is not None:
        b.grad.add_(dy2.sum(0))
        return None
    return dy2.sum(0).to(b.dtype)


class GatherLinearFn(torch.autograd.Function):

    @staticmethod
    def forward(ctx, x, weight, gathered, accumulate_into_grad):
        from .gemm import gemm_tn_gather
        ctx.save_for_backward(x, weight)
        ctx.has_bias = False
        ctx.accumulate = bool(accumulate_into_grad)
        ctx.weight_ref = weight
        ctx.bias_ref = None
        x2 = x.reshape(-1, x.shape[-1])
        return gemm_tn_gather(x2, weight.detach(), gathered).view(*x.shape[:-1], weight.shape[0])

    @staticmethod
    def backward(ctx, dy):
        dx, dw, _db, _ = _linear_backward(ctx, dy)
        return dx, dw, None, None


def linear(x: torch.Tensor, weight: torch.Tensor, bias: Optional[torch.Tensor] = None, accumulate_into_grad: bool = True,
           gathered=None, fp8: bool = False) -> torch.Tensor:
    if fp8 and gathered is None and torch.is_grad_enabled() and (weight.requires_grad or x.requires_grad):
        from .fp8 import Fp8LinearFn, fp8_supported
        if fp8_supported(x, weight, bias):
            return Fp8LinearFn.apply(x, weight, bias, accumulate_into_grad)
    if gathered is not None and bias is None and x.is_cuda:
        if torch.is_grad_enabled() and (weight.requires_grad or x.requires_grad):
            return GatherLinearFn.apply(x, weight, gathered, accumulate_into_grad)
        from .gemm import gemm_tn_gather
        x2 = x.reshape(-1, x.shape[-1])
        return gemm_tn_gather(x2, weight.detach(), gathered).view(*x.shape[:-1], weight.shape[0])
    if torch.is_grad_enabled() and (weight.requires_grad or x.requires_grad):
        return LinearFn.apply(x, weight, bias, accumulate_into_grad)
    return F.linear(x, weight, bias)
```

Before: 387,100.

## Fuse SwiGLU and RoPE into GEMM epilogues, fuse dSwiGLU into down-proj dgrad

Adds fused GEMM epilogue variants to the wgmma kernel. The gate/up projection now emits the SwiGLU activation alongside its output, the QKV projection applies rotary embedding in registers before storing, and the down-projection dgrad computes the SwiGLU backward directly from the loaded gate/up tile. The goal is to remove separate elementwise kernels and their HBM round trips for swiglu, rope and swiglu_bwd. In exchange the epilogues get heavier, with extra TMA loads and register pressure, and correctness depends on shape checks in gemm_fused_ok.

```diff
diff --git a/acco_b200/csrc/bindings.cpp b/acco_b200/csrc/bindings.cpp
--- a/acco_b200/csrc/bindings.cpp
+++ b/acco_b200/csrc/bindings.cpp
@@ -31,6 +31,11 @@
                   int M, int N, int K, int accumulate, int bn_req, int splits_req, int pm_req, int pn_req, int msub_req, int sms, cudaStream_t st);
 int acco_gemm_tn_gather(const void* x, const void* w_local, void* y, int M, int N, int K, const void* const* peers, int n_peers,
                         const int* tile_owner, uint32_t* flags, uint32_t* epoch, uint32_t* done, int sms, cudaStream_t st);
+int acco_gemm_tn_swiglu(const void* x, const void* w, void* gu, void* act, int M, int N, int K, int sms, cudaStream_t st);
+int acco_gemm_tn_rope(const void* x, const void* w, void* y, const float* cos_t, const float* sin_t, int rope_S, int rope_cols, int M, int N,
+                      int K, int sms, cudaStream_t st);
+int acco_gemm_nn_dswiglu(const void* dy, const void* w, const void* gu, void* dgu, int M, int N, int K, int sms, cudaStream_t st);
+int acco_gemm_fused_ok(int epi, int M, int N, int K, int rope_cols, int sms);
 long long acco_gemm_map_encodes();
 int acco_gemm_max_clusters(int cl, int sms);
 void acco_gemm_set_debug(unsigned long long* buf);
@@ -414,6 +419,48 @@
     return y;
 }
 
+bool gemm_fused_ok(int64_t mode, int64_t M, int64_t N, int64_t K, int64_t rope_cols) {
+    return acco_gemm_fused_ok((int)mode, (int)M, (int)N, (int)K, (int)rope_cols, sm_count()) == 1;
+}
+
+std::vector<torch::Tensor> gemm_swiglu(torch::Tensor x, torch::Tensor w) {
+    check_bf16(x, "x"); check_bf16(w, "w");
+    TORCH_CHECK(x.dim() == 2 && w.dim() == 2 && x.size(1) == w.size(1), "gemm_swiglu: x [M, K], w [N, K]");
+    const c10::cuda::CUDAGuard guard(x.device());
+    const int64_t M = x.size(0), K = x.size(1), N = w.size(0);
+    auto gu = torch::empty({M, N}, x.options());
+    auto act = torch::empty({M, N / 2}, x.options());
+    const int rc = acco_gemm_tn_swiglu(x.data_ptr(), w.data_ptr(), gu.data_ptr(), act.data_ptr(), (int)M, (int)N, (int)K, sm_count(), stream());
+    TORCH_CHECK(rc == 0, "gemm_swiglu launch failed, code ", rc, " (M=", M, " N=", N, " K=", K, ")");
+    return {gu, act};
+}
+
+torch::Tensor gemm_dswiglu(torch::Tensor dy, torch::Tensor w, torch::Tensor gu) {
+    check_bf16(dy, "dy"); check_bf16(w, "w"); check_bf16(gu, "gu");
+    TORCH_CHECK(dy.dim() == 2 && w.dim() == 2 && gu.dim() == 2 && dy.size(1) == w.size(0) && gu.size(0) == dy.size(0) &&
+                gu.size(1) == 2 * w.size(1), "gemm_dswiglu: dy [M, K], w [K, I], gu [M, 2 I]");
+    const c10::cuda::CUDAGuard guard(dy.device());
+    const int64_t M = dy.size(0), K = dy.size(1), N = w.size(1);
+    auto dgu = torch::empty_like(gu);
+    const int rc = acco_gemm_nn_dswiglu(dy.data_ptr(), w.data_ptr(), gu.data_ptr(), dgu.data_ptr(), (int)M, (int)N, (int)K, sm_count(), stream());
+    TORCH_CHECK(rc == 0, "gemm_dswiglu launch failed, code ", rc, " (M=", M, " N=", N, " K=", K, ")");
+    return dgu;
+}
+
+torch::Tensor gemm_rope(torch::Tensor x, torch::Tensor w, torch::Tensor cos_t, torch::Tensor sin_t, int64_t rope_S, int64_t rope_cols) {
+    check_bf16(x, "x"); check_bf16(w, "w"); check_f32(cos_t, "cos"); check_f32(sin_t, "sin");
+    TORCH_CHECK(x.dim() == 2 && w.dim() == 2 && x.size(1) == w.size(1), "gemm_rope: x [M, K], w [N, K]");
+    TORCH_CHECK(cos_t.dim() == 2 && cos_t.size(0) >= rope_S && cos_t.size(1) == 32 && sin_t.sizes() == cos_t.sizes(),
+                "gemm_rope: cos/sin tables must be [>= rope_S, 32]");
+    const c10::cuda::CUDAGuard guard(x.device());
+    const int64_t M = x.size(0), K = x.size(1), N = w.size(0);
+    auto y = torch::empty({M, N}, x.options());
+    const int rc = acco_gemm_tn_rope(x.data_ptr(), w.data_ptr(), y.data_ptr(), cos_t.data_ptr<float>(), sin_t.data_ptr<float>(), (int)rope_S,
+                                     (int)rope_cols, (int)M, (int)N, (int)K, sm_count(), stream());
+    TORCH_CHECK(rc == 0, "gemm_rope launch failed, code ", rc, " (M=", M, " N=", N, " K=", K, ")");
+    return y;
+}
+
 std::vector<torch::Tensor> fp8_quantize(torch::Tensor t, bool e5m2, bool rowmajor, bool transposed) {
     check_bf16(t, "t");
     TORCH_CHECK(t.dim() == 2 && t.size(0) % 16 == 0 && t.size(1) % 16 == 0 && t.numel() > 0, "fp8_quantize: t must be [R, C] with R, C multiples of 16");
@@ -567,6 +614,10 @@
     m.def("gemm_tn", &gemm_tn);
     m.def("gemm", &gemm);
     m.def("gemm_choose", &gemm_choose);
+    m.def("gemm_fused_ok", &gemm_fused_ok);
+    m.def("gemm_swiglu", &gemm_swiglu);
+    m.def("gemm_rope", &gemm_rope);
+    m.def("gemm_dswiglu", &gemm_dswiglu);
     m.def("fp8_quantize", &fp8_quantize);
     m.def("gemm_fp8", &gemm_fp8);
     m.def("gemm_map_encodes", &gemm_map_encodes);
diff --git a/acco_b200/csrc/gemm_wgmma.cu b/acco_b200/csrc/gemm_wgmma.cu
--- a/acco_b200/csrc/gemm_wgmma.cu
+++ b/acco_b200/csrc/gemm_wgmma.cu
@@ -47,7 +47,15 @@
     unsigned long long* dbg;
     const float* inv_scale_a;
     const float* inv_scale_b;
+    const float* rope_cos;
+    const float* rope_sin;
+    int rope_S, rope_cols;
+    CUtensorMap map_act;
 };
+
+constexpr int EPI_STORE = 0, EPI_SWIGLU = 1, EPI_ROPE = 2, EPI_DSWIGLU = 3;
+
+__device__ __forceinline__ float bf16_round(float x) { return __bfloat162float(__float2bfloat16_rn(x)); }
 
 constexpr int OP_BF16 = 0, OP_E4M3 = 1, OP_E5M2 = 2;
 
@@ -106,9 +114,12 @@
     else wgmma_m64n64k32_f8<OP == OP_E5M2>(acc, da, db, scale_d);
 }
 
-template <int BN, int A_MN, int B_MN, int OP>
+template <int BN, int A_MN, int B_MN, int OP, int EPI = EPI_STORE>
 __device__ __forceinline__ void gemm_body(const Params& P) {
     static_assert(OP == OP_BF16 || (A_MN == 0 && B_MN == 0), "FP8 wgmma has no transpose: both operands K-major");
+    static_assert(EPI == EPI_STORE || (OP == OP_BF16 && A_MN == 0 && B_MN == (EPI == EPI_DSWIGLU)),
+                  "fused epilogues: bf16, K-major A; B K-major (forward) or MN-major (dgrad)");
+    static_assert(EPI != EPI_SWIGLU || BN >= 128, "SwiGLU epilogue: 64-wide act sub-tiles");
     constexpr int BKE = OP ? 2 * BK : BK;
     extern __shared__ uint8_t smem_raw[];
     if (threadIdx.x == 0) stamp(P, 0);
@@ -206,6 +217,10 @@
                             if (mc_b) tma_load_2d_mc(bmap, &full_bar[stage], sb + c * MN_CHUNK_BYTES, n0 + c * 64, kb * BKE, mask_b);
                             else tma_load_2d(bmap, &full_bar[stage], sb + c * MN_CHUNK_BYTES, n0 + c * 64, kb * BKE);
                         }
+                    } else if constexpr (EPI == EPI_SWIGLU) {
+                        const int nh = n_blk * (BN / 2);
+                        tma_load_2d(bmap, &full_bar[stage], sb, kb * BKE, nh);
+                        tma_load_2d(bmap, &full_bar[stage], sb + (BN / 2) * 128, kb * BKE, P.N / 2 + nh);
                     } else {
                         if (mc_b) tma_load_2d_mc(bmap, &full_bar[stage], sb + b_off * 128, kb * BKE, n0 + b_off, mask_b);
                         else tma_load_2d(bmap, &full_bar[stage], sb, kb * BKE, n0);
@@ -239,6 +254,8 @@
             else mbar_arrive(&empty_bar[s]);
         };
         constexpr int NSUB = BN / 64;
+        constexpr int NOUT = EPI == EPI_SWIGLU ? NSUB + NSUB / 2 : NSUB;
+        int out_par = 0;
         constexpr int NPRE = NSUB < 2 ? NSUB : 2;
         uint8_t* epi = epi_smem + cw * 2 * EPI_BUF_BYTES;
         uint64_t* cbar = c_bar + cw * 2;
@@ -249,6 +266,12 @@
             if (NSUB == 1) bulk_wait_read<0>();
             else bulk_wait_read<1>();
         };
+        auto load_gu_pair = [&](const Unit& u, int s) {
+            const int c0 = u.n_blk * BN + s * 64, r0 = u.mb * BM + cw * 64;
+            mbar_expect_tx(&cbar[0], (uint32_t)(2 * EPI_BUF_BYTES));
+            tma_load_2d(&P.map_act, &cbar[0], epi, c0, r0);
+            tma_load_2d(&P.map_act, &cbar[0], epi + EPI_BUF_BYTES, P.N + c0, r0);
+        };
         auto load_c_sub = [&](const Unit& u, int s) {
             mbar_expect_tx(&cbar[s & 1], (uint32_t)EPI_BUF_BYTES);
             tma_load_2d(&P.map_d, &cbar[s & 1], epi + (s & 1) * EPI_BUF_BYTES, u.n_blk * BN + s * 64, u.mb * BM + cw * 64);
@@ -293,6 +316,12 @@
                 if (load_c && kb == u.kb0 && tid == 0) {
                     bulk_wait_read<0>();
                     for (int s = 0; s < NPRE; ++s) load_c_sub(u, s);
+                }
+                if constexpr (EPI == EPI_DSWIGLU) {
+                    if (kb == u.kb0 && tid == 0) {
+                        bulk_wait_read<0>();
+                        load_gu_pair(u, 0);
+                    }
                 }
                 if constexpr (OP != OP_BF16) {
                     wgmma_wait<0>();
@@ -319,9 +348,50 @@
             const int colb = u.n_blk * BN + 2 * (lane & 3);
             const bool bias_on = P.bias != nullptr && u.kb0 == 0;
 #pragma unroll
-            for (int s = 0; s < NSUB; ++s) {
-                uint8_t* buf = epi + (s & 1) * EPI_BUF_BYTES;
-                const uint32_t buf_addr = row_addr + (uint32_t)((s & 1) * EPI_BUF_BYTES);
+            for (int s = 0; s < NOUT; ++s) {
+                if constexpr (EPI == EPI_DSWIGLU) {
+                    if (s > 0 && tid == 0) {
+                        bulk_wait_read<0>();
+                        load_gu_pair(u, s);
+                    }
+                    mbar_wait(&cbar[0], c_phase & 1u);
+                    c_phase ^= 1u;
+#pragma unroll
+                    for (int jj = 0; jj < 8; ++jj) {
+                        const uint32_t ga = row_addr + (uint32_t)((jj ^ (lane >> 2)) << 4);
+#pragma unroll
+                        for (int h = 0; h < 2; ++h) {
+                            const uint32_t g_addr = ga + h * 8 * 128, u_addr = g_addr + EPI_BUF_BYTES;
+                            const uint32_t gv = ld_shared_u32(g_addr), uv = ld_shared_u32(u_addr);
+                            const float2 g2 = __bfloat1622float2(*reinterpret_cast<const __nv_bfloat162*>(&gv));
+                            const float2 u2 = __bfloat1622float2(*reinterpret_cast<const __nv_bfloat162*>(&uv));
+                            float dg[2], du[2];
+#pragma unroll
+                            for (int e = 0; e < 2; ++e) {
+                                const float fd = bf16_round(acc[4 * (s * 8 + jj) + 2 * h + e]);
+                                const float fg = e ? g2.y : g2.x, fu = e ? u2.y : u2.x;
+                                const float sg = 1.f / (1.f + __expf(-fg));
+                                const float silu = fg * sg;
+                                dg[e] = fd * fu * sg * (1.f + fg * (1.f - sg));
+                                du[e] = fd * silu;
+                            }
+                            st_shared_u32(g_addr, pack_bf16x2(dg[0], dg[1]));
+                            st_shared_u32(u_addr, pack_bf16x2(du[0], du[1]));
+                        }
+                    }
+                    fence_async_smem();
+                    named_barrier(bar_id, 128);
+                    if (tid == 0) {
+                        const int c0 = u.n_blk * BN + s * 64;
+                        tma_store_2d(&P.map_d, epi, c0, m0);
+                        tma_store_2d(&P.map_d, epi + EPI_BUF_BYTES, P.N + c0, m0);
+                        bulk_commit();
+                    }
+                    continue;
+                }
+                const int bsel = (EPI == EPI_SWIGLU && (NOUT & 1)) ? ((s + out_par) & 1) : (s & 1);
+                uint8_t* buf = epi + bsel * EPI_BUF_BYTES;
+                const uint32_t buf_addr = row_addr + (uint32_t)(bsel * EPI_BUF_BYTES);
                 if (load_c) {
                     if (s >= NPRE && tid == 0) {
                         wait_buffer_free();
@@ -333,43 +403,98 @@
                     if (tid == 0) wait_buffer_free();
                     named_barrier(bar_id, 128);
                 }
-#pragma unroll
-                for (int jj = 0; jj < 8; ++jj) {
-                    const int j = s * 8 + jj;
-                    const int col = colb + 8 * j;
-                    float b0 = 0.f, b1 = 0.f;
-                    if (bias_on && col < P.N) {
-                        const float2 f = __bfloat1622float2(*reinterpret_cast<const __nv_bfloat162*>(P.bias + col));
-                        b0 = f.x; b1 = f.y;
-                    }
-                    const uint32_t chunk_addr = buf_addr + (uint32_t)((jj ^ (lane >> 2)) << 4);
-#pragma unroll
-                    for (int h = 0; h < 2; ++h) {
-                        const uint32_t dst = chunk_addr + h * 8 * 128;
-                        float v0, v1;
-                        if constexpr (OP != OP_BF16) {
-                            v0 = acc[4 * j + 2 * h] * out_scale + b0;
-                            v1 = acc[4 * j + 2 * h + 1] * out_scale + b1;
-                        } else {
-                            v0 = acc[4 * j + 2 * h] + b0;
-                            v1 = acc[4 * j + 2 * h + 1] + b1;
+                if constexpr (EPI != EPI_STORE) {
+                    if (EPI == EPI_ROPE && u.n_blk * BN + s * 64 < P.rope_cols) {
+#pragma unroll
+                        for (int h = 0; h < 2; ++h) {
+                            const int pos = (m0 + warp * 16 + (lane >> 2) + 8 * h) % P.rope_S;
+                            const float* cp = P.rope_cos + (size_t)pos * 32 + 2 * (lane & 3);
+                            const float* sp = P.rope_sin + (size_t)pos * 32 + 2 * (lane & 3);
+#pragma unroll
+                            for (int jj = 0; jj < 4; ++jj) {
+                                const float2 c2 = __ldg(reinterpret_cast<const float2*>(cp + 8 * jj));
+                                const float2 s2 = __ldg(reinterpret_cast<const float2*>(sp + 8 * jj));
+#pragma unroll
+                                for (int e = 0; e < 2; ++e) {
+                                    const float c = e ? c2.y : c2.x, sn = e ? s2.y : s2.x;
+                                    float& p1 = acc[4 * (s * 8 + jj) + 2 * h + e];
+                                    float& p2 = acc[4 * (s * 8 + jj + 4) + 2 * h + e];
+                                    const float x1 = bf16_round(p1), x2 = bf16_round(p2);
+                                    p1 = __fmaf_rn(x1, c, -__fmul_rn(x2, sn));
+                                    p2 = __fmaf_rn(x2, c, __fmul_rn(x1, sn));
+                                }
+                            }
                         }
-                        if (load_c) {
-                            const uint32_t cv = ld_shared_u32(dst);
-                            const float2 c = __bfloat1622float2(*reinterpret_cast<const __nv_bfloat162*>(&cv));
-                            v0 += c.x; v1 += c.y;
+                    }
+#pragma unroll
+                    for (int jj = 0; jj < 8; ++jj) {
+                        const uint32_t chunk_addr = buf_addr + (uint32_t)((jj ^ (lane >> 2)) << 4);
+#pragma unroll
+                        for (int h = 0; h < 2; ++h) {
+                            float vv[2];
+#pragma unroll
+                            for (int e = 0; e < 2; ++e) {
+                                if (EPI == EPI_SWIGLU && s >= NSUB) {
+                                    const int j = (s - NSUB) * 8 + jj;
+                                    const float g = bf16_round(acc[4 * j + 2 * h + e]);
+                                    const float up = bf16_round(acc[4 * (j + BN / 16) + 2 * h + e]);
+                                    const float sg = 1.f / (1.f + __expf(-g));
+                                    vv[e] = g * sg * up;
+                                } else {
+                                    vv[e] = acc[4 * (s * 8 + jj) + 2 * h + e];
+                                }
+                            }
+                            st_shared_u32(chunk_addr + h * 8 * 128, pack_bf16x2(vv[0], vv[1]));
                         }
-                        st_shared_u32(dst, pack_bf16x2(v0, v1));
+                    }
+                } else {
+#pragma unroll
+                    for (int jj = 0; jj < 8; ++jj) {
+                        const int j = s * 8 + jj;
+                        const int col = colb + 8 * j;
+                        float b0 = 0.f, b1 = 0.f;
+                        if (bias_on && col < P.N) {
+                            const float2 f = __bfloat1622float2(*reinterpret_cast<const __nv_bfloat162*>(P.bias + col));
+                            b0 = f.x; b1 = f.y;
+                        }
+                        const uint32_t chunk_addr = buf_addr + (uint32_t)((jj ^ (lane >> 2)) << 4);
+#pragma unroll
+                        for (int h = 0; h < 2; ++h) {
+                            const uint32_t dst = chunk_addr + h * 8 * 128;
+                            float v0, v1;
+                            if constexpr (OP != OP_BF16) {
+                                v0 = acc[4 * j + 2 * h] * out_scale + b0;
+                                v1 = acc[4 * j + 2 * h + 1] * out_scale + b1;
+                            } else {
+                                v0 = acc[4 * j + 2 * h] + b0;
+                                v1 = acc[4 * j + 2 * h + 1] + b1;
+                            }
+                            if (load_c) {
+                                const uint32_t cv = ld_shared_u32(dst);
+                                const float2 c = __bfloat1622float2(*reinterpret_cast<const __nv_bfloat162*>(&cv));
+                                v0 += c.x; v1 += c.y;
+                            }
+                            st_shared_u32(dst, pack_bf16x2(v0, v1));
+                        }
                     }
                 }
                 fence_async_smem();
                 named_barrier(bar_id, 128);
                 if (tid == 0) {
-                    if (P.atomic) tma_reduce_add_2d(&P.map_d, buf, u.n_blk * BN + s * 64, m0);
-                    else tma_store_2d(&P.map_d, buf, u.n_blk * BN + s * 64, m0);
+                    if constexpr (EPI == EPI_SWIGLU) {
+                        const int nh = u.n_blk * (BN / 2);
+                        if (s < NSUB / 2) tma_store_2d(&P.map_d, buf, nh + s * 64, m0);
+                        else if (s < NSUB) tma_store_2d(&P.map_d, buf, P.N / 2 + nh + (s - NSUB / 2) * 64, m0);
+                        else tma_store_2d(&P.map_act, buf, nh + (s - NSUB) * 64, m0);
+                    } else if (P.atomic) {
+                        tma_reduce_add_2d(&P.map_d, buf, u.n_blk * BN + s * 64, m0);
+                    } else {
+                        tma_store_2d(&P.map_d, buf, u.n_blk * BN + s * 64, m0);
+                    }
                     bulk_commit();
                 }
             }
+            if constexpr (EPI == EPI_SWIGLU) out_par ^= NOUT & 1;
         }
         if (tid == 0) bulk_wait<0>();
         if (cw == 0 && tid == 0) stamp(P, 7);
@@ -397,6 +522,11 @@
 template <int BN, int OP>
 __global__ void __launch_bounds__(THREADS, 1) gemm_fp8_kernel(const __grid_constant__ Params P) {
     gemm_body<BN, 0, 0, OP>(P);
+}
+
+template <int BN, int EPI>
+__global__ void __launch_bounds__(THREADS, 1) gemm_fused_kernel(const __grid_constant__ Params P) {
+    gemm_body<BN, 0, EPI == EPI_DSWIGLU ? 1 : 0, OP_BF16, EPI>(P);
 }
 
 typedef CUresult (*EncodeFn)(CUtensorMap*, CUtensorMapDataType, cuuint32_t, void*, const cuuint64_t*, const cuuint64_t*, const cuuint32_t*,
@@ -500,6 +630,13 @@
     if (bn == 128) return op == OP_E5M2 ? gemm_fp8_kernel<128, OP_E5M2> : gemm_fp8_kernel<128, OP_E4M3>;
     return op == OP_E5M2 ? gemm_fp8_kernel<64, OP_E5M2> : gemm_fp8_kernel<64, OP_E4M3>;
 }
+static KernelFn fused_kernel_for(int bn, int epi) {
+    if (epi == EPI_SWIGLU) return bn == 256 ? gemm_fused_kernel<256, EPI_SWIGLU> : bn == 128 ? gemm_fused_kernel<128, EPI_SWIGLU> : nullptr;
+    if (epi == EPI_ROPE)
+        return bn == 256 ? gemm_fused_kernel<256, EPI_ROPE> : bn == 128 ? gemm_fused_kernel<128, EPI_ROPE> : gemm_fused_kernel<64, EPI_ROPE>;
+    if (epi == EPI_DSWIGLU) return bn == 256 ? gemm_fused_kernel<256, EPI_DSWIGLU> : bn == 128 ? gemm_fused_kernel<128, EPI_DSWIGLU> : nullptr;
+    return nullptr;
+}
 
 static int g_pm = 0, g_pn = 0;
 static unsigned long long* g_dbg = nullptr;
@@ -515,6 +652,10 @@
         for (int bn : {64, 128})
             for (int op : {OP_E4M3, OP_E5M2})
                 if (cudaFuncSetAttribute(fp8_kernel_for(bn, op), cudaFuncAttributeMaxDynamicSharedMemorySize, SMEM_BYTES) != cudaSuccess) rc = -4;
+        for (int bn : {64, 128, 256})
+            for (int epi : {EPI_SWIGLU, EPI_ROPE, EPI_DSWIGLU})
+                if (KernelFn f = fused_kernel_for(bn, epi))
+                    if (cudaFuncSetAttribute(f, cudaFuncAttributeMaxDynamicSharedMemorySize, SMEM_BYTES) != cudaSuccess) rc = -4;
         const char* e;
         if ((e = getenv("ACCO_GEMM_CLUSTER")) && e[0] && e[1] == ',') { g_pm = e[0] - '0'; g_pn = e[2] - '0'; }
         if ((e = getenv("ACCO_GEMM_PDL")) && e[0] == '0') g_pdl = 0;
@@ -627,9 +768,25 @@
     uint32_t* done;
 };
 
+struct EpiArgs {
+    int mode;
+    void* act;
+    const float* cos;
+    const float* sin;
+    int rope_S, rope_cols;
+};
+
+static int fused_unsupported(int epi, const Config& c, int N, int rope_cols) {
+    if (c.splits != 1 || c.pm != 1 || c.pn != 1) return 1;
+    if (epi == EPI_SWIGLU) return (c.bn < 128 || N % 2 || (N / 2) % (c.bn / 2)) ? 1 : 0;
+    if (epi == EPI_ROPE) return (rope_cols < 0 || rope_cols % 64 || rope_cols > N) ? 1 : 0;
+    if (epi == EPI_DSWIGLU) return (c.bn < 128 || N % 64) ? 1 : 0;
+    return 1;
+}
+
 static int launch(const void* a, long long lda, int a_mn, const void* b, long long ldb, int b_mn, void* d, long long ldd, const void* bias, int M,
                   int N, int K, int accumulate, int bn_req, int splits_req, int pm_req, int pn_req, int msub_req, const GatherArgs* ga, int sms,
-                  cudaStream_t st, int op = OP_BF16, const float* inv_a = nullptr, const float* inv_b = nullptr) {
+                  cudaStream_t st, int op = OP_BF16, const float* inv_a = nullptr, const float* inv_b = nullptr, const EpiArgs* ep = nullptr) {
     if (M <= 0 || N <= 0 || K <= 0) return -1;
     if ((lda % 8) || (ldb % 8) || (ldd % 8) || (N % 8)) return -1;
     const int eb = op ? 1 : 2, bke = op ? 2 * BK : BK;
@@ -653,12 +810,19 @@
     if ((bn_req > 0 && bn != bn_req) || (pm_req > 0 && pm != pm_req) || (pn_req > 0 && pn != pn_req)) return -1;
     if (b_mn ? ((bn / 64) % pm != 0) : ((bn / pm) % 8 != 0)) return -1;
     if (a_mn && (BM / 64) % pn != 0) return -1;
+    const int epi = ep ? ep->mode : EPI_STORE;
+    if (epi != EPI_STORE) {
+        if (op || a_mn || b_mn != (epi == EPI_DSWIGLU) || gather || accumulate || bias || ldd != (epi == EPI_DSWIGLU ? 2LL * N : N)) return -1;
+        if (fused_unsupported(epi, cfgc, N, ep->rope_cols)) return -7;
+        if ((epi == EPI_SWIGLU || epi == EPI_DSWIGLU) && (!ep->act || ((uintptr_t)ep->act % 16))) return -1;
+        if (epi == EPI_ROPE && (!ep->cos || !ep->sin || ep->rope_S <= 0)) return -1;
+    }
     Params P;
     if (a_mn) rc = make_map(&P.map_a, a, (uint64_t)M, (uint64_t)K, (uint64_t)lda, 64, BK);
     else rc = make_map_typed(&P.map_a, a, (uint64_t)K, (uint64_t)M, (uint64_t)lda, bke, (uint32_t)(BM / pn), eb);
     if (rc) return rc;
     if (b_mn) rc = make_map(&P.map_b, b, (uint64_t)N, (uint64_t)K, (uint64_t)ldb, 64, BK);
-    else rc = make_map_typed(&P.map_b, b, (uint64_t)K, (uint64_t)N, (uint64_t)ldb, bke, (uint32_t)(bn / pm), eb);
+    else rc = make_map_typed(&P.map_b, b, (uint64_t)K, (uint64_t)N, (uint64_t)ldb, bke, (uint32_t)(epi == EPI_SWIGLU ? bn / 2 : bn / pm), eb);
     if (rc) return rc;
     for (int i = 0; i < MAX_PEERS; ++i) {
         if (gather && i < ga->n_peers) {
@@ -668,8 +832,21 @@
             P.map_b_peer[i] = P.map_b;
         }
     }
-    rc = make_map(&P.map_d, d, (uint64_t)N, (uint64_t)M, (uint64_t)ldd, 64, 64);
+    rc = make_map(&P.map_d, d, (uint64_t)(epi == EPI_DSWIGLU ? 2 * N : N), (uint64_t)M, (uint64_t)ldd, 64, 64);
     if (rc) return rc;
+    if (epi == EPI_SWIGLU) {
+        rc = make_map(&P.map_act, ep->act, (uint64_t)(N / 2), (uint64_t)M, (uint64_t)(N / 2), 64, 64);
+        if (rc) return rc;
+    } else if (epi == EPI_DSWIGLU) {
+        rc = make_map(&P.map_act, ep->act, (uint64_t)(2 * N), (uint64_t)M, (uint64_t)(2 * N), 64, 64);
+        if (rc) return rc;
+    } else {
+        P.map_act = P.map_d;
+    }
+    P.rope_cos = epi == EPI_ROPE ? ep->cos : nullptr;
+    P.rope_sin = epi == EPI_ROPE ? ep->sin : nullptr;
+    P.rope_S = epi == EPI_ROPE ? ep->rope_S : 1;
+    P.rope_cols = epi == EPI_ROPE ? ep->rope_cols : 0;
     P.bias = (const __nv_bfloat16*)bias;
     P.out = (__nv_bfloat16*)d;
     P.ldd = ldd;
@@ -729,7 +906,7 @@
     }
     cfg.attrs = attr;
     cfg.numAttrs = na;
-    return (int)cudaLaunchKernelEx(&cfg, op ? fp8_kernel_for(bn, op) : kernel_for(bn, a_mn, b_mn), P);
+    return (int)cudaLaunchKernelEx(&cfg, epi != EPI_STORE ? fused_kernel_for(bn, epi) : op ? fp8_kernel_for(bn, op) : kernel_for(bn, a_mn, b_mn), P);
 }
 
 }
@@ -752,6 +929,30 @@
                                  cudaStream_t st) {
     return acco_gemm::launch(a, lda, 0, b, ldb, 0, d, ldd, bias, M, N, K, accumulate, bn_req, splits_req, 0, 0, 0, nullptr, sms, st,
                              a_e5m2 ? acco_gemm::OP_E5M2 : acco_gemm::OP_E4M3, inv_a, inv_b);
+}
+
+extern "C" int acco_gemm_tn_swiglu(const void* x, const void* w, void* gu, void* act, int M, int N, int K, int sms, cudaStream_t st) {
+    acco_gemm::EpiArgs ep{acco_gemm::EPI_SWIGLU, act, nullptr, nullptr, 1, 0};
+    return acco_gemm::launch(x, K, 0, w, K, 0, gu, N, nullptr, M, N, K, 0, 0, 0, 0, 0, 0, nullptr, sms, st, acco_gemm::OP_BF16, nullptr, nullptr, &ep);
+}
+
+extern "C" int acco_gemm_tn_rope(const void* x, const void* w, void* y, const float* cos_t, const float* sin_t, int rope_S, int rope_cols, int M,
+                                 int N, int K, int sms, cudaStream_t st) {
+    acco_gemm::EpiArgs ep{acco_gemm::EPI_ROPE, nullptr, cos_t, sin_t, rope_S, rope_cols};
+    return acco_gemm::launch(x, K, 0, w, K, 0, y, N, nullptr, M, N, K, 0, 0, 0, 0, 0, 0, nullptr, sms, st, acco_gemm::OP_BF16, nullptr, nullptr, &ep);
+}
+
+extern "C" int acco_gemm_nn_dswiglu(const void* dy, const void* w, const void* gu, void* dgu, int M, int N, int K, int sms, cudaStream_t st) {
+    acco_gemm::EpiArgs ep{acco_gemm::EPI_DSWIGLU, const_cast<void*>(gu), nullptr, nullptr, 1, 0};
+    return acco_gemm::launch(dy, K, 0, w, N, 1, dgu, 2LL * N, nullptr, M, N, K, 0, 0, 0, 0, 0, 0, nullptr, sms, st, acco_gemm::OP_BF16, nullptr, nullptr,
+                             &ep);
+}
+
+extern "C" int acco_gemm_fused_ok(int epi, int M, int N, int K, int rope_cols, int sms) {
+    acco_gemm::init_once();
+    const int b_mn = epi == acco_gemm::EPI_DSWIGLU ? 1 : 0;
+    const acco_gemm::Config c = acco_gemm::choose_config(M, N, K, 0, b_mn, 0, sms, 0, 0, acco_gemm::g_pm, acco_gemm::g_pn);
+    return (N % 8 == 0 && K % 8 == 0 && !acco_gemm::fused_unsupported(epi, c, N, rope_cols)) ? 1 : 0;
 }
 
 extern "C" int acco_gemm_tile_n() { return acco_gemm::BN_MAX; }
diff --git a/acco_b200/models/llama.py b/acco_b200/models/llama.py
--- a/acco_b200/models/llama.py
+++ b/acco_b200/models/llama.py
@@ -187,12 +187,16 @@
                 n = ops.rmsnorm(h, layer.input_layernorm.weight, eps)
             else:
                 n, h = ops.add_rmsnorm(branch, h, layer.input_layernorm.weight, eps)
-            qkv = ops.linear(n, layer.self_attn.qkv_proj, gathered=self._gw(layer.self_attn.qkv_proj), fp8=fp8)
-            att = ops.rope_causal_attention(qkv, cos, sin, B, S, Hq, Hk, D, seg=seg)
+            qkv_w, gw = layer.self_attn.qkv_proj, self._gw(layer.self_attn.qkv_proj)
+            qkv = ops.linear_rope(n, qkv_w, cos, sin, T if seg is not None else S, (Hq + Hk) * D, gathered=gw, fp8=fp8)
+            rotated = qkv is not None
+            if not rotated:
+                qkv = ops.linear(n, qkv_w, gathered=gw, fp8=fp8)
+            att = ops.rope_causal_attention(qkv, cos, sin, B, S, Hq, Hk, D, seg=seg, rotated=rotated)
             o = ops.linear(att, layer.self_attn.o_proj, gathered=self._gw(layer.self_attn.o_proj), fp8=fp8)
             n, h = ops.add_rmsnorm(o, h, layer.post_attention_layernorm.weight, eps)
-            gu = ops.linear(n, layer.mlp.gate_up_proj, gathered=self._gw(layer.mlp.gate_up_proj), fp8=fp8)
-            branch = ops.linear(ops.swiglu(gu), layer.mlp.down_proj, gathered=self._gw(layer.mlp.down_proj), fp8=fp8)
+            branch = ops.llama_mlp(n, layer.mlp.gate_up_proj, layer.mlp.down_proj, gathered_gu=self._gw(layer.mlp.gate_up_proj),
+                                   gathered_down=self._gw(layer.mlp.down_proj), fp8=fp8)
         if branch is None:
             n = ops.rmsnorm(h, self.model.norm.weight, eps)
         else:
diff --git a/acco_b200/ops/__init__.py b/acco_b200/ops/__init__.py
--- a/acco_b200/ops/__init__.py
+++ b/acco_b200/ops/__init__.py
@@ -89,7 +89,7 @@
 from .embedding import embedding
 from .activation import swiglu, swiglu_ref, gelu_new, gelu_new_ref
 from .cross_entropy import softmax_cross_entropy, softmax_cross_entropy_ref
-from .linear import linear, LinearFn
+from .linear import linear, LinearFn, linear_rope, llama_mlp
 from .attention import causal_attention, causal_attention_ref, rope_causal_attention, packed_causal_attention, segment_starts
 from .adam import fused_adamw_shard, grad_sumsq
 
@@ -101,7 +101,7 @@
     "rope_qkv", "rope_qkv_ref", "apply_rope_ref", "rope_tables", "embedding",
     "swiglu", "swiglu_ref",
     "softmax_cross_entropy", "softmax_cross_entropy_ref",
-    "linear", "LinearFn",
+    "linear", "LinearFn", "linear_rope", "llama_mlp",
     "causal_attention", "causal_attention_ref", "rope_causal_attention", "packed_causal_attention", "segment_starts",
     "fused_adamw_shard", "grad_sumsq",
 ]
diff --git a/acco_b200/ops/attention.py b/acco_b200/ops/attention.py
--- a/acco_b200/ops/attention.py
+++ b/acco_b200/ops/attention.py
@@ -271,11 +271,11 @@
 class _RopeAttentionFn(torch.autograd.Function):
 
     @staticmethod
-    def forward(ctx, qkv, cos, sin, B, S, Hq, Hk, D, rope=True, scale=None, window=None, seg=None):
+    def forward(ctx, qkv, cos, sin, B, S, Hq, Hk, D, rope=True, scale=None, window=None, seg=None, rotated=False):
         from . import count_launch, load_ext
         C = load_ext(required=True)
         rb, rs = (1, B * S) if (rope and seg is not None) else (B, S)
-        if rope:
+        if rope and not rotated:
             C.rope_qkv_inplace(qkv, cos, sin, rb, rs, Hq + Hk, Hq + 2 * Hk, D, False)
             count_launch("rope_qkv")
         sc = (1.0 / math.sqrt(D)) if scale is None else float(scale)
@@ -314,7 +314,7 @@
             count_launch("attn_bwd" if seg is None else "attn_bwd_seg", 2)
             dqkv = C.rope_pack_bwd(dq.to(torch.bfloat16).view(rb, rs, Hq, D), dk.view(rb, rs, Hk, D), dv.view(rb, rs, Hk, D), cos, sin)
             count_launch("rope_pack_bwd")
-            return (dqkv,) + (None,) * 11
+            return (dqkv,) + (None,) * 12
         out, q, k, v = ctx.inner
         ctx.inner = None
         do = dout.reshape(B, S, Hq, D).transpose(1, 2)
@@ -325,19 +325,20 @@
             dq, dk, dv = (t.reshape(rb, rs, t.shape[2], D) for t in (dq, dk, dv))
         dqkv = C.rope_pack_bwd(dq, dk, dv, cos, sin)
         count_launch("rope_pack_bwd")
-        return (dqkv,) + (None,) * 11
+        return (dqkv,) + (None,) * 12
 
 
 def rope_causal_attention(qkv: torch.Tensor, cos: torch.Tensor, sin: torch.Tensor, B: int, S: int, Hq: int, Hk: int, D: int,
-                          seg: Optional[torch.Tensor] = None) -> torch.Tensor:
+                          seg: Optional[torch.Tensor] = None, rotated: bool = False) -> torch.Tensor:
     from . import use_kernels
     from .rope import rope_qkv_ref
     if use_kernels(qkv):
         if seg is not None or (torch.is_grad_enabled() and qkv.requires_grad):
-            return _RopeAttentionFn.apply(qkv, cos, sin, B, S, Hq, Hk, D, True, None, None, seg)
+            return _RopeAttentionFn.apply(qkv, cos, sin, B, S, Hq, Hk, D, True, None, None, seg, rotated)
         from . import count_launch, load_ext
-        load_ext(required=True).rope_qkv_inplace(qkv, cos, sin, B, S, Hq + Hk, Hq + 2 * Hk, D, False)
-        count_launch("rope_qkv")
+        if not rotated:
+            load_ext(required=True).rope_qkv_inplace(qkv, cos, sin, B, S, Hq + Hk, Hq + 2 * Hk, D, False)
+            count_launch("rope_qkv")
         x = qkv.view(B, S, Hq + 2 * Hk, D)
         out = _sdpa(x[:, :, :Hq].transpose(1, 2), x[:, :, Hq:Hq + Hk].transpose(1, 2), x[:, :, Hq + Hk:].transpose(1, 2), None, Hk != Hq)
         return out.transpose(1, 2).reshape(B * S, Hq * D)
diff --git a/acco_b200/ops/linear.py b/acco_b200/ops/linear.py
--- a/acco_b200/ops/linear.py
+++ b/acco_b200/ops/linear.py
@@ -50,8 +50,9 @@
     return st
 
 
-def _linear_backward(ctx, dy):
-    x, weight = ctx.saved_tensors
+def _linear_backward(ctx, dy, x=None, weight=None):
+    if x is None:
+        x, weight = ctx.saved_tensors
     dy2 = dy.reshape(-1, dy.shape[-1])
     x2 = x.reshape(-1, x.shape[-1])
     if dy2.dtype != weight.dtype or x2.dtype != dy2.dtype:
@@ -126,6 +127,98 @@
         return dx, dw, None, None
 
 
+def _fused_ok(mode: int, x2: torch.Tensor, weight: torch.Tensor, rope_cols: int = 0) -> bool:
+    from . import load_ext
+    return (_tc(x2, weight) and x2.is_contiguous() and weight.is_contiguous() and x2.data_ptr() % 16 == 0 and weight.data_ptr() % 16 == 0
+            and load_ext(required=True).gemm_fused_ok(mode, x2.shape[0], weight.shape[0], x2.shape[1], rope_cols))
+
+
+def _save_linear(ctx, weight, accumulate_into_grad):
+    ctx.has_bias = False
+    ctx.accumulate = bool(accumulate_into_grad)
+    ctx.weight_ref = weight
+    ctx.bias_ref = None
+
+
+class _LlamaMLPFn(torch.autograd.Function):
+
+    @staticmethod
+    def forward(ctx, x, w_gu, w_down, accumulate_into_grad):
+        from . import count_launch, load_ext
+        from .gemm import gemm_tn
+        x2 = x.reshape(-1, x.shape[-1])
+        gu, act = load_ext(required=True).gemm_swiglu(x2, w_gu.detach())
+        count_launch("gemm_swiglu")
+        y = gemm_tn(act, w_down.detach())
+        ctx.save_for_backward(x, w_gu, w_down, gu, act)
+        ctx.accumulate = bool(accumulate_into_grad)
+        return y.view(*x.shape[:-1], w_down.shape[0])
+
+    @staticmethod
+    def backward(ctx, dy):
+        from types import SimpleNamespace
+        from . import count_launch, load_ext
+        C = load_ext(required=True)
+        x, w_gu, w_down, gu, act = ctx.saved_tensors
+        dy2 = dy.reshape(-1, dy.shape[-1]).contiguous()
+        T, I, H = dy2.shape[0], act.shape[1], dy2.shape[1]
+        if _tc(dy2, w_down) and C.gemm_fused_ok(3, T, I, H, 0):
+            dgu = C.gemm_dswiglu(dy2, w_down.detach(), gu)
+            count_launch("gemm_dswiglu")
+        else:
+            from .gemm import gemm_nn
+            dgu = C.swiglu_bwd(gemm_nn(dy2, w_down.detach()), gu)
+            count_launch("swiglu_bwd")
+        need = ctx.needs_input_grad
+        down = SimpleNamespace(needs_input_grad=(False, need[2], False), accumulate=ctx.accumulate, weight_ref=w_down, has_bias=False)
+        _, dw_down, _, _ = _linear_backward(down, dy2, act, w_down)
+        gate_up = SimpleNamespace(needs_input_grad=(need[0], need[1], False), accumulate=ctx.accumulate, weight_ref=w_gu, has_bias=False)
+        dx, dw_gu, _, _ = _linear_backward(gate_up, dgu, x, w_gu)
+        return dx, dw_gu, dw_down, None
+
+
+def llama_mlp(x: torch.Tensor, w_gu: torch.Tensor, w_down: torch.Tensor, accumulate_into_grad: bool = True, gathered_gu=None,
+              gathered_down=None, fp8: bool = False) -> torch.Tensor:
+    from .activation import swiglu
+    x2 = x.reshape(-1, x.shape[-1])
+    if not fp8 and gathered_gu is None and gathered_down is None and _fused_ok(1, x2, w_gu) and _tc(x2, w_down):
+        return _LlamaMLPFn.apply(x, w_gu, w_down, accumulate_into_grad)
+    act = swiglu(linear(x, w_gu, accumulate_into_grad=accumulate_into_grad, gathered=gathered_gu, fp8=fp8))
+    return linear(act, w_down, accumulate_into_grad=accumulate_into_grad, gathered=gathered_down, fp8=fp8)
+
+
+class _LinearRopeFn(torch.autograd.Function):
+
+    @staticmethod
+    def forward(ctx, x, weight, cos, sin, rope_rows, rope_cols, accumulate_into_grad):
+        from . import count_launch, load_ext
+        ctx.save_for_backward(x, weight)
+        _save_linear(ctx, weight, accumulate_into_grad)
+        x2 = x.reshape(-1, x.shape[-1])
+        y = load_ext(required=True).gemm_rope(x2, weight.detach(), cos, sin, rope_rows, rope_cols)
+        count_launch("gemm_rope")
+        return y.view(*x.shape[:-1], weight.shape[0])
+
+    @staticmethod
+    def backward(ctx, dy):
+        dx, dw, _db, _ = _linear_backward(ctx, dy)
+        return dx, dw, None, None, None, None, None
+
+
+def linear_rope(x: torch.Tensor, weight: torch.Tensor, cos: torch.Tensor, sin: torch.Tensor, rope_rows: int, rope_cols: int,
+                accumulate_into_grad: bool = True, gathered=None, fp8: bool = False) -> Optional[torch.Tensor]:
+    x2 = x.reshape(-1, x.shape[-1])
+    if (fp8 or gathered is not None or not cos.is_cuda or cos.dtype != torch.float32 or cos.dim() != 2 or cos.shape[1] != 32
+            or not cos.is_contiguous() or not sin.is_contiguous() or not _fused_ok(2, x2, weight, rope_cols)):
+        return None
+    if torch.is_grad_enabled() and (weight.requires_grad or x.requires_grad):
+        return _LinearRopeFn.apply(x, weight, cos, sin, int(rope_rows), int(rope_cols), accumulate_into_grad)
+    from . import count_launch, load_ext
+    y = load_ext(required=True).gemm_rope(x2, weight.detach(), cos, sin, int(rope_rows), int(rope_cols))
+    count_launch("gemm_rope")
+    return y.view(*x.shape[:-1], weight.shape[0])
+
+
 def linear(x: torch.Tensor, weight: torch.Tensor, bias: Optional[torch.Tensor] = None, accumulate_into_grad: bool = True,
            gathered=None, fp8: bool = False) -> torch.Tensor:
     if fp8 and gathered is None and torch.is_grad_enabled() and (weight.requires_grad or x.requires_grad):
```

After: 399,700, median of 6. 3.2% higher.
